# LongmaoTeamTf/deep_recommenders

Hardware: AMD Instinct MI355X
Metric: examples/sec/node DeepFM (26 sparse feats, 10M vocab, dim 64) (higher is better)
Workload: dtype f32; 1 GPU; DeepFM Criteo-shape synthetic training step (BASELINE.json configs[2]): 26 sparse + 13 dense, 10000000 vocab/field hashed on device, dim 64, DNN [256, 32]+[1] relu, sigmoid-CE, fused SGD; batch 65536 per GPU, ids uniform; tables on one GPU (66.6 GB); gemm_split=f16x2, global_batch=65536, parallelism=single, per_kernel_events=False

## Files before the change

deep_recommenders_amd/csrc/bf3_planes.hip:

```cpp
#include "bf3_rs_core.h"

namespace {

using namespace drrs;

constexpr int NWAVES = 8;
constexpr int NTHREADS = 64 * NWAVES;

struct NtArgs {
    const __bf16* A; int64_t a_ps, a_ld;
    const __bf16* B; int64_t b_ps, b_ld;
    int64_t M; int32_t N; int32_t K;
    float* C; int64_t ldc;
    const float* bias; int32_t act;
    const float* mask; int64_t ld_mask;
};


template <int NW, int DBG = 0>
__global__ __launch_bounds__(64 * NW, NW / 4) void bf3_gemm_nt_pipe_kernel(NtArgs g) {
    constexpr int BM = 128, BN = 128, NS = 3;
    constexpr int WN = 4, WM = NW / WN, TM = BM / (32 * WM);
    constexpr int A_PLANE = BM * 64, B_PLANE = BN * 64;
    constexpr int STAGE = 3 * (A_PLANE + B_PLANE);
    constexpr int KB_A = 3 * A_PLANE / 1024, PW = STAGE / 1024 / NW;
    constexpr int P1 = (PW + 1) / 2, P0 = PW - P1;
    static_assert((NW == 8 || NW == 16) && PW * NW * 1024 == STAGE, "wave layout");
    __shared__ __attribute__((aligned(1024))) unsigned char smem[NS * STAGE];

    const int tid = threadIdx.x, lane = tid & 63;
    const int wave = __builtin_amdgcn_readfirstlane(tid >> 6);
    const int wm = wave / WN, wn = wave % WN;
    const int l31 = lane & 31, hi = lane >> 5;

    const int tiles_n = (g.N + BN - 1) / BN;
    const int tiles_m = (int)((g.M + BM - 1) / BM);
    const int ntiles = tiles_m * tiles_n;
    const int nk = g.K / BK;
    if ((int)blockIdx.x >= ntiles) return;
    const int my_tiles = (ntiles - (int)blockIdx.x + (int)gridDim.x - 1) / (int)gridDim.x;
    const int total = my_tiles * nk;

    const unsigned lds0 = (unsigned)(uintptr_t)(lds_ptr_t)smem;
    const int sw = (l31 >> 2) & 3;
    unsigned a_addr[2], b_addr[2];
#pragma unroll
    for (int ks = 0; ks < 2; ++ks) {
        a_addr[ks] = lds0 + (wm * 32 * TM + l31) * 64 + (((2 * ks + hi) ^ sw) << 4);
        b_addr[ks] = lds0 + 3 * A_PLANE + (wn * 32 + l31) * 64 + (((2 * ks + hi) ^ sw) << 4);
    }

    const __bf16* src[PW];
    int p_tile = blockIdx.x, p_kt = 0, p_stage = 0;
    auto setup_src = [&](int tile) {
        const int lid = xcd_remap(tile, ntiles);
        const int64_t m0 = (int64_t)(lid / tiles_n) * BM;
        const int n0 = (lid % tiles_n) * BN;
#pragma unroll
        for (int i = 0; i < PW; ++i) {
            const int j = wave + NW * i;
            const bool is_a = j < KB_A;
            const int jj = is_a ? j : j - KB_A;
            const int plane = jj >> 3, rb = jj & 7;
            const int row = rb * 16 + (lane >> 2);
            const int c = (lane & 3) ^ ((row >> 2) & 3);
            int64_t grow = (is_a ? m0 : (int64_t)n0) + row;
            const int64_t lim = is_a ? g.M : (int64_t)g.N;
            grow = grow < lim ? grow : lim - 1;
            src[i] = is_a ? g.A + plane * g.a_ps + grow * g.a_ld + c * 8 : g.B + plane * g.b_ps + grow * g.b_ld + c * 8;
        }
    };
    auto issue_piece = [&](int i) {
        lds_dma16(src[i], smem + p_stage * STAGE + (wave + NW * i) * 1024);
        if constexpr (!(DBG & 4)) src[i] += BK;
    };
    auto advance = [&]() {
        p_stage = p_stage == NS - 1 ? 0 : p_stage + 1;
        if (++p_kt == nk) {
            p_kt = 0;
            p_tile += gridDim.x;
            if (p_tile < ntiles) setup_src(p_tile);
        }
    };
// ... 391 lines not shown
        const float4* s4 = reinterpret_cast<const float4*>(src);
        const int64_t stride = (int64_t)gridDim.x * blockDim.x;
        int64_t i = (int64_t)blockIdx.x * blockDim.x + threadIdx.x;
        for (; i + 3 * stride < nv; i += 4 * stride) {
            const float4 v0 = s4[i], v1 = s4[i + stride], v2 = s4[i + 2 * stride], v3 = s4[i + 3 * stride];
            take4(v0); take4(v1); take4(v2); take4(v3);
        }
        for (; i < nv; i += stride) take4(s4[i]);
        for (int64_t j = (nv << 2) + (int64_t)blockIdx.x * blockDim.x + threadIdx.x; j < n; j += stride) m = max(m, __float_as_uint(fabsf(src[j])));
    } else {
        const bool vec = al16 && (ld & 3) == 0;
        const int cv = vec ? (C >> 2) : 0;
        for (int64_t r = blockIdx.x; r < R; r += gridDim.x) {
            const float* row = src + r * ld;
            for (int c = threadIdx.x; c < cv; c += blockDim.x) take4(reinterpret_cast<const float4*>(row)[c]);
            for (int c = (cv << 2) + threadIdx.x; c < C; c += blockDim.x) m = max(m, __float_as_uint(fabsf(row[c])));
        }
    }
#pragma unroll
    for (int o = 32; o > 0; o >>= 1) m = max(m, (uint32_t)__shfl_xor((int)m, o, 64));
    __shared__ uint32_t wm[4];
    if ((threadIdx.x & 63) == 0) wm[threadIdx.x >> 6] = m;
    __syncthreads();
    if (threadIdx.x == 0) {
        m = max(max(wm[0], wm[1]), max(wm[2], wm[3]));
        if (m > __hip_atomic_load(amax, __ATOMIC_RELAXED, __HIP_MEMORY_SCOPE_AGENT)) atomicMax(amax, m);
    }
}

__global__ __launch_bounds__(256) void h2_split_kernel(const float* __restrict__ src, int64_t ld_src, int64_t R, int32_t C,
                                                       _Float16* __restrict__ planes, int64_t ps, int64_t ldp, int64_t r0,
                                                       int64_t c0, int32_t transpose, const uint32_t* __restrict__ amax) {
    float sc, inv;
    h2_scale_of(amax[0], sc, inv);
    h2_mode_on();
    const int64_t total = R * C, stride = (int64_t)gridDim.x * blockDim.x;
    if (!transpose && (C & 3) == 0 && (ldp & 3) == 0 && (c0 & 3) == 0 && (ld_src & 3) == 0 && (reinterpret_cast<uintptr_t>(src) & 15) == 0 &&
        (reinterpret_cast<uintptr_t>(planes) & 7) == 0 && (ps & 3) == 0 && total < (int64_t)0x7fffffff) {
        typedef _Float16 f16x4 __attribute__((ext_vector_type(4)));
        typedef float f32x4 __attribute__((ext_vector_type(4)));
        const unsigned cq = (unsigned)C >> 2, tq = (unsigned)(total >> 2);
        for (unsigned i = blockIdx.x * blockDim.x + threadIdx.x; i < tq; i += (unsigned)stride) {
            const unsigned r = i / cq, c = (i - r * cq) << 2;
            const f32x4 v = *reinterpret_cast<const f32x4*>(src + (int64_t)r * ld_src + c) * sc;
            const f16x4 h = __builtin_convertvector(v, f16x4);
            const f16x4 l = __builtin_convertvector(v - __builtin_convertvector(h, f32x4), f16x4);
            const int64_t off = (r0 + r) * ldp + c0 + c;
            *reinterpret_cast<f16x4*>(planes + off) = h;
            *reinterpret_cast<f16x4*>(planes + ps + off) = l;
        }
        return;
    }
    for (int64_t i = (int64_t)blockIdx.x * blockDim.x + threadIdx.x; i < total; i += stride) {
        int64_t r, c, off;
        if (!transpose) { r = i / C; c = i - r * C; off = (r0 + r) * ldp + c0 + c; }
        else { c = i / R; r = i - c * R; off = (r0 + c) * ldp + c0 + r; }
        const float v = src[r * ld_src + c] * sc;
        const _Float16 h = (_Float16)v;
        planes[off] = h;
        planes[ps + off] = (_Float16)(v - (float)h);
    }
}

constexpr int H2_REFRESH_PARTS = 256;
__global__ __launch_bounds__(256) void h2_amax_parts_kernel(const float* __restrict__ src, int64_t ld, int64_t R, int32_t C,
                                                            uint32_t* __restrict__ parts) {
    uint32_t m = 0u;
    const int64_t total = R * (int64_t)C, stride = (int64_t)gridDim.x * blockDim.x;
    for (int64_t i = (int64_t)blockIdx.x * blockDim.x + threadIdx.x; i < total; i += stride) {
        const int64_t r = i / C;
        m = max(m, __float_as_uint(fabsf(src[r * ld + (i - r * C)])));
    }
#pragma unroll
    for (int o = 32; o > 0; o >>= 1) m = max(m, (uint32_t)__shfl_xor((int)m, o, 64));
    __shared__ uint32_t wm[4];
    if ((threadIdx.x & 63) == 0) wm[threadIdx.x >> 6] = m;
    __syncthreads();
    if (threadIdx.x == 0) parts[blockIdx.x] = max(max(wm[0], wm[1]), max(wm[2], wm[3]));
}
__global__ __launch_bounds__(256) void h2_split_both_kernel(const float* __restrict__ src, int64_t ld, int64_t R, int32_t C,
                                                            _Float16* __restrict__ w, int64_t w_ps, int64_t w_ld,
                                                            _Float16* __restrict__ wt, int64_t wt_ps, int64_t wt_ld,
                                                            const uint32_t* __restrict__ parts, int32_t nparts, uint32_t* __restrict__ amax) {
    uint32_t m = (int)threadIdx.x < nparts ? parts[threadIdx.x] : 0u;
#pragma unroll
    for (int o = 32; o > 0; o >>= 1) m = max(m, (uint32_t)__shfl_xor((int)m, o, 64));
    __shared__ uint32_t wm[4];
    if ((threadIdx.x & 63) == 0) wm[threadIdx.x >> 6] = m;
    __syncthreads();
    m = max(max(wm[0], wm[1]), max(wm[2], wm[3]));
    if (blockIdx.x == 0 && threadIdx.x == 0) amax[0] = m;
    float sc, inv;
    h2_scale_of(m, sc, inv);
    h2_mode_on();
    const int64_t total = R * (int64_t)C, stride = (int64_t)gridDim.x * blockDim.x;
    for (int64_t i = (int64_t)blockIdx.x * blockDim.x + threadIdx.x; i < 2 * total; i += stride) {
        int64_t r, c, off;
        _Float16* dst;
        int64_t ps;
        if (i < total) { r = i / C; c = i - r * C; off = r * w_ld + c; dst = w; ps = w_ps; }
        else { const int64_t j = i - total; c = j / R; r = j - c * R; off = c * wt_ld + r; dst = wt; ps = wt_ps; }
        const float v = src[r * ld + c] * sc;
        const _Float16 h = (_Float16)v;
        dst[off] = h;
        dst[ps + off] = (_Float16)(v - (float)h);
    }
}

__global__ __launch_bounds__(256) void bf3_join_kernel(const __bf16* __restrict__ planes, int64_t ps, int64_t ldp, int64_t R,
                                                       int32_t C, float* __restrict__ dst, int64_t ld_dst) {
    const int64_t total = R * C, stride = (int64_t)gridDim.x * blockDim.x;
    for (int64_t i = (int64_t)blockIdx.x * blockDim.x + threadIdx.x; i < total; i += stride) {
        const int64_t r = i / C;
        const int c = (int)(i - r * C);
        const int64_t off = r * ldp + c;
        dst[r * ld_dst + c] = bf3::join(planes[off], planes[ps + off], planes[2 * ps + off]);
    }
}

}

extern "C" int dr_bf3_split(const float* src, int64_t ld_src, int64_t R, int32_t C, void* planes, int64_t plane_stride,
                            int64_t ld_planes, int64_t row_offset, int64_t col_offset, int32_t transpose,
                            dr_stream_t stream) {
    if (R < 0 || C < 0 || ld_src < C || row_offset < 0 || col_offset < 0 || ld_planes <= 0 || plane_stride <= 0) return DR_EINVAL;
    if (R == 0 || C == 0) return DR_OK;
    if (!src || !planes) return DR_EINVAL;
    if (!transpose && col_offset + C > ld_planes) return DR_EINVAL;
    if (transpose && col_offset + R > ld_planes) return DR_EINVAL;
    hipLaunchKernelGGL(bf3_split_kernel, dim3(dr_grid_for(R * ((C + 3) / 4), 256)), dim3(256), 0, dr_s(stream), src, ld_src, R, C,
                       static_cast<__bf16*>(planes), plane_stride, ld_planes, row_offset, col_offset, transpose);
    DR_CHECK_LAUNCH();
    return DR_OK;
}

extern "C" int dr_bf3_join(const void* planes, int64_t plane_stride, int64_t ld_planes, int64_t R, int32_t C, float* dst,
                           int64_t ld_dst, dr_stream_t stream) {
    if (R < 0 || C < 0 || ld_planes < C || ld_dst < C || plane_stride <= 0) return DR_EINVAL;
    if (R == 0 || C == 0) return DR_OK;
    if (!planes || !dst) return DR_EINVAL;
    hipLaunchKernelGGL(bf3_join_kernel, dim3(dr_grid_for(R * C, 256)), dim3(256), 0, dr_s(stream),
                       static_cast<const __bf16*>(planes), plane_stride, ld_planes, R, C, dst, ld_dst);
    DR_CHECK_LAUNCH();
    return DR_OK;
}

extern "C" int dr_bf3_gemm_nt(const void* a_planes, int64_t a_plane_stride, int64_t a_ld, const void* b_planes,
                              int64_t b_plane_stride, int64_t b_ld, int64_t M, int32_t N, int32_t K, const float* bias,
                              int32_t act, const float* mask, int64_t ld_mask, float* C, int64_t ldc, dr_stream_t stream) {
    if (M < 0 || N <= 0 || K <= 0 || (K % BK) != 0 || act < 0 || act > 1) return DR_EINVAL;
    if (M == 0) return DR_OK;
    if (!planes_ok(a_planes, a_plane_stride, a_ld) || !planes_ok(b_planes, b_plane_stride, b_ld) || !C) return DR_EINVAL;
    if (a_ld < K || b_ld < K || ldc < N || (mask != nullptr && ld_mask < N)) return DR_EINVAL;
    NtArgs g{static_cast<const __bf16*>(a_planes), a_plane_stride, a_ld, static_cast<const __bf16*>(b_planes), b_plane_stride, b_ld,
             M, N, K, C, ldc, bias, act, mask, ld_mask};
    const int64_t tiles = ((M + 127) / 128) * ((N + 127) / 128);
    if (tiles > 0x7fffffff) return DR_EINVAL;
    const int grid = (int)(tiles < 256 ? tiles : 256);
    hipLaunchKernelGGL((bf3_gemm_nt_pipe_kernel<16>), dim3(grid), dim3(1024), 0, dr_s(stream), g);
    DR_CHECK_LAUNCH();
    return DR_OK;
}

extern "C" int64_t dr_bf3_gemm_tn_workspace_bytes(int64_t R, int32_t F, int32_t N) {
    if (R <= 0 || F <= 0 || N <= 0) return 0;
    return (int64_t)tn_split_for(R, F, N, 128, 256) * F * N * (int64_t)sizeof(float);
}

extern "C" int dr_bf3_gemm_tn(const void* x_planes, int64_t x_plane_stride, int64_t x_ld, const void* y_planes,
                              int64_t y_plane_stride, int64_t y_ld, int64_t R, int32_t F, int32_t N, float scale, float* dst,
                              int64_t ld_dst, const float* y_colsum, float* dstb, void* workspace, int64_t workspace_bytes,
                              dr_stream_t stream) {
    if (R <= 0 || F <= 0 || N <= 0) return DR_EINVAL;
    if (!planes_ok(x_planes, x_plane_stride, x_ld) || !planes_ok(y_planes, y_plane_stride, y_ld) || !dst || !workspace) return DR_EINVAL;
    if (x_ld < F || y_ld < N || ld_dst < N) return DR_EINVAL;
    if (workspace_bytes < dr_bf3_gemm_tn_workspace_bytes(R, F, N)) return DR_EINVAL;
    TnArgs g{static_cast<const __bf16*>(x_planes), x_plane_stride, x_ld, static_cast<const __bf16*>(y_planes), y_plane_stride, y_ld,
             R, F, N, 0, 0, static_cast<float*>(workspace)};
    int split = tn_split_for(R, F, N, 128, 256);
    const int64_t rpad = (R + BK - 1) / BK * BK;
    g.per = ((rpad + split - 1) / split + BK - 1) / BK * BK;
    g.split = (int32_t)((rpad + g.per - 1) / g.per);
    const int64_t tiles = (int64_t)((F + 127) / 128) * ((N + 255) / 256) * g.split;
    const int grid = (int)(tiles < 256 ? tiles : 256);
    hipLaunchKernelGGL((bf3_gemm_tn_kernel<2, 4>), dim3(grid), dim3(NTHREADS), 0, dr_s(stream), g);
    hipLaunchKernelGGL(bf3_splitk_reduce_kernel, dim3(dr_grid_for((int64_t)F * N, 256)), dim3(256), 0, dr_s(stream), g.partial,
                       g.split, (int64_t)F, N, scale, dst, ld_dst, y_colsum, dstb);
    DR_CHECK_LAUNCH();
    return DR_OK;
// ... 40 lines not shown
```

deep_recommenders_amd/csrc/emb_plan.hip:

```cpp
#include "dr_common.h"
#include "hash_i64.h"
#include <atomic>

namespace {

constexpr int CH = 32;
constexpr uint32_t EMPTY = 0xFFFFFFFFu;
constexpr uint32_t DUPBIT = 0x80000000u;
constexpr int SMALL_CAP = 16384;
constexpr int RADIX_BITS = 8, RADIX = 1 << RADIX_BITS;
constexpr int NBK = RADIX, CAPB = 128;
constexpr int LDS_TAB_MAX_LOG = 15;
constexpr int RADIX_CHUNK = 1664, RADIX_MAX_BLOCKS = 1024;
constexpr int MARK_BLOCKS = 512, MARK_MAX_CHUNK = 8192;
static_assert(NBK * CAPB >= SMALL_CAP, "buckets must hold the largest SMALL list");

std::atomic<int> g_small_limit{SMALL_CAP};

struct Ctrl {
    int32_t large;
    int32_t pad[3];
    int32_t bcnt[NBK];
};

// ... 467 lines not shown
    __syncthreads();
    const uint32_t base_row = rmin;
    int passes = 0;
    if (cnt > 1 && rmax > rmin) passes = (int)((bits_for_dev(rmax - rmin) + RADIX_BITS - 1) / RADIX_BITS);
    if (passes & 1) {
        for (int32_t i = t; i < cnt; i += LG_T) dst[i] = src[i];
        uint64_t* x = src; src = dst; dst = x;
        __syncthreads();
    }
    for (int p = 0; p < passes; ++p) {
        const uint32_t shift = (uint32_t)(p * RADIX_BITS);
        if (t < RADIX) running[t] = 0;
        __syncthreads();
        for (int32_t i = t; i < cnt; i += LG_T)
            atomicAdd(&running[(((uint32_t)(src[i] >> 24) - base_row) >> shift) & (RADIX - 1)], 1u);
        __syncthreads();
        {
            const uint32_t mine = t < RADIX ? running[t] : 0u;
            for (int o = 1; o < RADIX; o <<= 1) {
                const uint32_t x = (t < RADIX && t >= o) ? running[t - o] : 0u;
                __syncthreads();
                if (t < RADIX) running[t] += x;
                __syncthreads();
            }
            if (t < RADIX) running[t] -= mine;
        }
        __syncthreads();
        for (int32_t base = 0; base < cnt; base += LG_T) {
            const int32_t i = base + t;
            const bool live = i < cnt;
            const uint64_t k = live ? src[i] : 0ull;
            scatter_step_1024(live, k, (((uint32_t)(k >> 24) - base_row) >> shift) & (RADIX - 1), running, wcnt, dst);
        }
        uint64_t* x = src; src = dst; dst = x;
    }
    for (int32_t base = 0; base < cnt; base += LG_T) {
        const int32_t i = base + t;
        const bool in = i < cnt;
        const uint64_t ck = in ? src[i] : ~0ull;
        const uint64_t k = ck >> 24;
        const int32_t gi = (int32_t)beg + i;
        const bool valid = in && k < num_rows;
        const bool seg_start = in && (i == 0 || (src[i - 1] >> 24) != k);
        const bool has_next = in && (i + 1 < cnt) && (src[i + 1] >> 24) == k;
        if (in) {
            const int32_t slot = (int32_t)(ck & 0xFFFFFFu);
            rows[gi] = k;
            slots[gi] = slot;
            flags[slot] = (valid && seg_start && !has_next) ? 1 : 0;
        }
        const bool head = valid && ((seg_start && has_next) || (!seg_start && (gi % CH) == 0 && i >= CH && (src[i - CH] >> 24) == k));
        if (t == 0) nh = 0;
        __syncthreads();
        const uint64_t bal = __ballot(head);
        int wbase = 0;
        const int leader = bal != 0 ? __ffsll((unsigned long long)bal) - 1 : 0;
        if (bal != 0 && lane == leader) wbase = atomicAdd(&nh, __popcll(bal));
        __syncthreads();
        if (t == 0) gbase = nh > 0 ? atomicAdd(dup_count, nh) : 0;
        __syncthreads();
        if (bal != 0) {
            wbase = __shfl(wbase, leader, 64);
            if (head) dup_heads[gbase + wbase + __popcll(bal & ((1ull << lane) - 1ull))] = gi;
        }
    }
}

}

extern "C" int32_t dr_emb_plan_set_small_limit(int32_t limit) {
    if (limit < 0) limit = 0;
    if (limit > SMALL_CAP) limit = SMALL_CAP;
    return g_small_limit.exchange(limit);
}

extern "C" int64_t dr_emb_sort_workspace_bytes(int64_t n) {
    if (n <= 0) return 256;
    return (int64_t)layout_for(n).total;
}

namespace {
int plan_small_front(const int64_t* raw, const uint64_t* col_buckets, int64_t* ids_out, int32_t* ids_t, const int64_t* ids, int64_t B,
                     int32_t F, const int64_t* row_base, int64_t num_rows, uint64_t* rows_y, uint64_t* keys_x, uint32_t* ghist,
                     uint32_t* tot, Ctrl* ctrl, int32_t* dup_count, hipStream_t s) {
    const int64_t n64 = B * F;
    const int32_t n = (int32_t)n64;
    const uint32_t mul = (uint32_t)((((uint64_t)RADIX) << 32) / (uint64_t)num_rows);
    int64_t sub = 64;
    while ((B + sub - 1) / sub > RADIX_MAX_BLOCKS) sub += 64;
    const int nbf = (int)((B + sub - 1) / sub);
    const int nbs = (nbf + FRONT_GROUP - 1) / FRONT_GROUP;
    const int64_t chunk = sub * FRONT_GROUP * F;
    if (chunk > 0x7fffffff) return DR_EINVAL;
    const bool trans = ids_t != nullptr;
    const size_t lds = (size_t)8 * (raw ? 3 : 1) * F + (trans ? (size_t)4 * 64 * (F + 1) : 0);
    if (raw) {
        if (trans)
            hipLaunchKernelGGL((plan_front_kernel<true, true>), dim3(nbf), dim3(256), lds, s, raw, B, F, col_buckets, ids_out, ids_t, row_base,
                               (uint64_t)num_rows, mul, (int32_t)sub, rows_y, ghist);
        else
            hipLaunchKernelGGL((plan_front_kernel<true, false>), dim3(nbf), dim3(256), lds, s, raw, B, F, col_buckets, ids_out, ids_t,
                               row_base, (uint64_t)num_rows, mul, (int32_t)sub, rows_y, ghist);
    } else {
        hipLaunchKernelGGL((plan_front_kernel<false, false>), dim3(nbf), dim3(256), lds, s, ids, B, F, col_buckets, ids_out, ids_t, row_base,
                           (uint64_t)num_rows, mul, (int32_t)sub, rows_y, ghist);
    }
    hipLaunchKernelGGL((radix_scan_kernel<true>), dim3(RADIX), dim3(256), 0, s, ghist, (int32_t)nbf, tot, ctrl, dup_count);
    hipLaunchKernelGGL(plan_scatter_kernel, dim3(nbs), dim3(LG_T), 0, s, rows_y, keys_x, n, mul, (int32_t)chunk, ghist, (int32_t)nbf, tot);
    return DR_OK;
}

int sort_slots_impl(const int64_t* raw, const uint64_t* col_buckets, int32_t* ids_t, const int64_t* ids, int64_t B, int32_t F,
                    const int64_t* row_base, int64_t num_rows, int64_t* sorted_rows, int32_t* sorted_slots, uint8_t* unique_flags,
                    int32_t* dup_heads, int32_t* dup_count, void* workspace, int64_t workspace_bytes, dr_stream_t stream) {
    if (B < 0 || F <= 0 || num_rows <= 0) return DR_EINVAL;
    const int64_t n64 = B * F;
    if (n64 == 0) return DR_OK;
    if (n64 > 0x7fffff00) return DR_EINVAL;
    if (!ids || !row_base || !sorted_rows || !sorted_slots || !unique_flags || !dup_heads || !dup_count || !workspace)
        return DR_EINVAL;
    if (workspace_bytes < dr_emb_sort_workspace_bytes(n64)) return DR_EINVAL;
    const int32_t n = (int32_t)n64;
    const Layout L = layout_for(n64);
    char* w = static_cast<char*>(workspace);
    uint64_t* keys_x = reinterpret_cast<uint64_t*>(w + L.keys_x);
    uint32_t* vals_x = reinterpret_cast<uint32_t*>(w + L.vals_x);
    uint64_t* blist = reinterpret_cast<uint64_t*>(w + L.blist);
    uint32_t* ghist = reinterpret_cast<uint32_t*>(w + L.ghist);
    uint32_t* tot = reinterpret_cast<uint32_t*>(w + L.tot);
    Ctrl* ctrl = reinterpret_cast<Ctrl*>(w + L.ctrl);
    uint64_t* rows_y = reinterpret_cast<uint64_t*>(sorted_rows);
    uint32_t* slots_y = reinterpret_cast<uint32_t*>(sorted_slots);
    hipStream_t s = dr_s(stream);
    const int grid = dr_grid_for(n, 256);
    const int nb = radix_blocks(n);

    const bool claimable = n64 <= (1 << 24) && num_rows < 0x7fffffffLL;
    const bool fused_front = raw != nullptr && claimable && F <= 64;
    if (raw && !fused_front) {
        int rc = dr_hash_bucket_i64(raw, B, F, col_buckets, const_cast<int64_t*>(ids), stream);
        if (rc == DR_OK && ids_t) rc = dr_ids_transpose_i32(ids, B, F, ids_t, stream);
        if (rc != DR_OK) return rc;
    }
    if (claimable) {
        int rc = plan_small_front(fused_front ? raw : nullptr, col_buckets, const_cast<int64_t*>(ids), fused_front ? ids_t : nullptr, ids, B,
                                  F, row_base, num_rows, rows_y, keys_x, ghist, tot, ctrl, dup_count, s);
        if (rc != DR_OK) return rc;
        static const hipError_t lds_optin = hipFuncSetAttribute(reinterpret_cast<const void*>(plan_lds_claim_kernel),
                                                                hipFuncAttributeMaxDynamicSharedMemorySize, 4 << LDS_TAB_MAX_LOG);
        if (lds_optin != hipSuccess) return DR_ELAUNCH;
        int log_tab = 12;
        while (log_tab < LDS_TAB_MAX_LOG && (1 << log_tab) < 2 * ((n + NBK - 1) / NBK)) ++log_tab;
        hipLaunchKernelGGL(plan_lds_claim_kernel, dim3(NBK), dim3(CLAIM_T), (size_t)4 << log_tab, s, keys_x, tot, (uint64_t)num_rows,
                           (int32_t)log_tab, unique_flags, blist, ctrl);
        hipLaunchKernelGGL(plan_bucket_sort_kernel, dim3(NBK), dim3(256), 0, s, blist, ctrl, (int32_t)g_small_limit.load(), rows_y,
                           sorted_slots, dup_heads, dup_count);
        hipLaunchKernelGGL(plan_large_kernel, dim3(NBK), dim3(LG_T), 0, s, keys_x, tot, (uint64_t)num_rows, n, rows_y, sorted_slots,
                           unique_flags, dup_heads, dup_count, ctrl);
        DR_CHECK_LAUNCH();
        return DR_OK;
    }
    if (hipMemsetAsync(dup_count, 0, 2 * sizeof(int32_t), s) != hipSuccess) return DR_ELAUNCH;
    const unsigned bits = bits_for((uint64_t)num_rows);
    const int passes = (int)((bits + RADIX_BITS - 1) / RADIX_BITS);
    uint64_t* kbuf[2] = {keys_x, rows_y};
    uint32_t* vbuf[2] = {vals_x, slots_y};
    int cur = (passes & 1) ? 0 : 1;
    hipLaunchKernelGGL(radix_make_keys_kernel, dim3(grid), dim3(256), 0, s, ids, n, F, row_base, (uint64_t)num_rows, kbuf[cur], vbuf[cur]);
    for (int p = 0; p < passes; ++p) {
        const uint32_t shift = (uint32_t)(p * RADIX_BITS);
        hipLaunchKernelGGL(radix_hist_kernel, dim3(nb), dim3(256), 0, s, kbuf[cur], n, shift, ghist);
        hipLaunchKernelGGL((radix_scan_kernel<false>), dim3(RADIX), dim3(256), 0, s, ghist, (int32_t)nb, tot, ctrl, dup_count);
        hipLaunchKernelGGL(radix_scatter_kernel, dim3(nb), dim3(256), 0, s, kbuf[cur], vbuf[cur], kbuf[cur ^ 1], vbuf[cur ^ 1], n, shift, ghist,
                           tot);
        cur ^= 1;
    }
    int mark_blocks = MARK_BLOCKS;
    while ((n + mark_blocks - 1) / mark_blocks > MARK_MAX_CHUNK) mark_blocks *= 2;
    hipLaunchKernelGGL(radix_mark_kernel, dim3(mark_blocks), dim3(256), 0, s, rows_y, sorted_slots, n, (uint64_t)num_rows, unique_flags, dup_heads,
                       dup_count);
    DR_CHECK_LAUNCH();
    return DR_OK;
}
}

extern "C" int dr_emb_sort_slots(const int64_t* ids, int64_t B, int32_t F, const int64_t* row_base, int64_t num_rows,
                                 int64_t* sorted_rows, int32_t* sorted_slots, uint8_t* unique_flags, int32_t* dup_heads,
                                 int32_t* dup_count, void* workspace, int64_t workspace_bytes, dr_stream_t stream) {
    return sort_slots_impl(nullptr, nullptr, nullptr, ids, B, F, row_base, num_rows, sorted_rows, sorted_slots, unique_flags, dup_heads,
                           dup_count, workspace, workspace_bytes, stream);
}

extern "C" int dr_hash_sort_slots(const int64_t* keys, int64_t B, int32_t F, const uint64_t* col_buckets, int64_t* ids_out,
                                  int32_t* ids_t_out, const int64_t* row_base, int64_t num_rows, int64_t* sorted_rows,
                                  int32_t* sorted_slots, uint8_t* unique_flags, int32_t* dup_heads, int32_t* dup_count, void* workspace,
                                  int64_t workspace_bytes, dr_stream_t stream) {
    if (!keys || !col_buckets || !ids_out) return DR_EINVAL;
    return sort_slots_impl(keys, col_buckets, ids_t_out, ids_out, B, F, row_base, num_rows, sorted_rows, sorted_slots, unique_flags,
                           dup_heads, dup_count, workspace, workspace_bytes, stream);
}
```

deep_recommenders_amd/csrc/emb_sorted.hip:

```cpp
#include <cstdlib>
#include "dr_common.h"
#include "tn_rs_reduce.h"
#include <hip/amd_detail/amd_hip_unsafe_atomics.h>
#include <cstring>

namespace {

constexpr int CH = 32;

#ifndef DR_K4_NT
#define DR_K4_NT 1
#endif
typedef float dr_f4v __attribute__((ext_vector_type(4)));
__device__ __forceinline__ float4 ld4_stream(const float* p) {
#if DR_K4_NT
    const dr_f4v v = __builtin_nontemporal_load(reinterpret_cast<const dr_f4v*>(p));
    return make_float4(v.x, v.y, v.z, v.w);
#else
    return *reinterpret_cast<const float4*>(p);
#endif
}
__device__ __forceinline__ void st4_stream(float* p, const float4 v) {
#if DR_K4_NT
    const dr_f4v w = {v.x, v.y, v.z, v.w};
// ... 242 lines not shown
        const bool exclusive = seg_start && (j >= n || rows[j < n ? j : n - 1] != k);
        float* dst = table + k * (uint64_t)D + sub * 4;
        if (ADAM) {
            if (live && seg_start) {
                if (dvalid) {
                    float4 t = *reinterpret_cast<const float4*>(dst);
                    float4 mt = *reinterpret_cast<const float4*>(ad.m + k * (uint64_t)D + sub * 4);
                    float4 vt = *reinterpret_cast<const float4*>(ad.v + k * (uint64_t)D + sub * 4);
                    t.x += adam_elem(g.x, mt.x, vt.x, ad); t.y += adam_elem(g.y, mt.y, vt.y, ad);
                    t.z += adam_elem(g.z, mt.z, vt.z, ad); t.w += adam_elem(g.w, mt.w, vt.w, ad);
                    wmax = amax4(wmax, t);
                    *reinterpret_cast<float4*>(dst) = t;
                    *reinterpret_cast<float4*>(ad.m + k * (uint64_t)D + sub * 4) = mt;
                    *reinterpret_cast<float4*>(ad.v + k * (uint64_t)D + sub * 4) = vt;
                }
                if (lin_w != nullptr && any_lin && sub == 0) {
                    float ml = ad.m_lin != nullptr ? ad.m_lin[k * ad.lin_stride] : 0.f, vl = ad.v_lin != nullptr ? ad.v_lin[k * ad.lin_stride] : 0.f;
                    lin_w[k] += adam_elem(dls, ml, vl, ad);
                    if (ad.m_lin != nullptr) { ad.m_lin[k * ad.lin_stride] = ml; ad.v_lin[k * ad.lin_stride] = vl; }
                }
            }
        } else if (live) {
            if (exclusive) {
                if (dvalid) {
                    float4 t = *reinterpret_cast<const float4*>(dst);
                    t.x = fmaf(scale, g.x, t.x); t.y = fmaf(scale, g.y, t.y);
                    t.z = fmaf(scale, g.z, t.z); t.w = fmaf(scale, g.w, t.w);
                    wmax = amax4(wmax, t);
                    *reinterpret_cast<float4*>(dst) = t;
                }
                if (lin_w != nullptr && any_lin && sub == 0) lin_w[k] = fmaf(scale, dls, lin_w[k]);
            } else if (det) {
                if (dvalid) *reinterpret_cast<float4*>(x_sorted + i * (int64_t)D + sub * 4) = g;
                if (any_lin && sub == 0 && j - i >= 2) x_sorted[(i + 1) * (int64_t)D] = dls;
            } else {
                if (dvalid && amax != nullptr) {
                    float4 o;
                    o.x = unsafeAtomicAdd(dst + 0, scale * g.x) + scale * g.x; o.y = unsafeAtomicAdd(dst + 1, scale * g.y) + scale * g.y;
                    o.z = unsafeAtomicAdd(dst + 2, scale * g.z) + scale * g.z; o.w = unsafeAtomicAdd(dst + 3, scale * g.w) + scale * g.w;
                    wmax = amax4(wmax, o);
                } else if (dvalid) {
                    unsafeAtomicAdd(dst + 0, scale * g.x); unsafeAtomicAdd(dst + 1, scale * g.y);
                    unsafeAtomicAdd(dst + 2, scale * g.z); unsafeAtomicAdd(dst + 3, scale * g.w);
                }
                if (lin_w != nullptr && any_lin && sub == 0) unsafeAtomicAdd(lin_w + k, scale * dls);
            }
        }
    }
    if (amax != nullptr) amax_commit(amax, wmax);
}

struct BwdSortedArgs {
    const int64_t* ids; const uint8_t* flags; int64_t B; int32_t F; const int64_t* row_base; int32_t D;
    const float* grad; int64_t ld; const float* concat; int64_t ldc; const float* sum_x; const float* d_fm_logit;
    const float* slot_lin; float scale; float* table; float* lin_w; float* lin_bias;
    const uint64_t* rows; const int32_t* slots; int64_t n; const int32_t* dup_heads; const int32_t* dup_count; uint64_t num_rows;
    float* x_sorted;
    int det;
    int skip_unique_lin;
    const float* lin_old_t;
    uint32_t* amax;
    int dups_only;
};
#ifndef DR_K4_MINWAVES
#define DR_K4_LB __launch_bounds__(256)
#else
#define DR_K4_LB __launch_bounds__(256, DR_K4_MINWAVES)
#endif
template <int LPR, int U, bool ADAM>
__global__ DR_K4_LB void emb_bwd_sorted_kernel(BwdSortedArgs a, AdamArgs ad, int grid_d) {
    if ((int)blockIdx.x < grid_d)
        emb_bwd_dups_body<LPR, ADAM>(blockIdx.x, grid_d, a.rows, a.slots, a.n, a.dup_heads, a.dup_count, a.F, a.D, a.num_rows, a.grad,
                                     a.ld, a.concat, a.ldc, a.sum_x, a.d_fm_logit, a.slot_lin, a.scale, a.table, a.lin_w, ad, a.x_sorted,
                                     a.det != 0, a.amax);
    else if (a.dups_only) {
        if (!ADAM && a.lin_bias != nullptr && a.d_fm_logit != nullptr) dr_block_sum_axpy(a.d_fm_logit, a.B, a.scale, a.lin_bias);
    } else
        emb_bwd_unique_body<LPR, U, ADAM>(blockIdx.x - grid_d, gridDim.x - grid_d, a.ids, a.flags, a.B, a.F, a.row_base, a.D, a.grad,
                                          a.ld, a.concat, a.ldc, a.sum_x, a.d_fm_logit, a.slot_lin, a.scale, a.table,
                                          a.skip_unique_lin ? nullptr : a.lin_w, a.lin_bias, ad, a.lin_old_t, a.amax);
}

template <int LPR>
__global__ __launch_bounds__(256) void emb_bwd_dups_apply_kernel(BwdSortedArgs a, drrs::TnRsApply ap, int grid_d) {
    const int bid = blockIdx.x;
    if (bid < grid_d)
        emb_bwd_dups_body<LPR, false>(bid, grid_d, a.rows, a.slots, a.n, a.dup_heads, a.dup_count, a.F, a.D, a.num_rows, a.grad, a.ld,
                                      a.concat, a.ldc, a.sum_x, a.d_fm_logit, a.slot_lin, a.scale, a.table, a.lin_w, AdamArgs{}, a.x_sorted,
                                      a.det != 0, a.amax);
    else if (bid == grid_d) {
        if (a.lin_bias != nullptr && a.d_fm_logit != nullptr) dr_block_sum_axpy(a.d_fm_logit, a.B, a.scale, a.lin_bias);
    } else
        drrs::tn_rs_reduce_ride(ap, bid - grid_d - 1, (int)gridDim.x - grid_d - 1, threadIdx.x);
}

template <int LPR>
__global__ __launch_bounds__(256) void emb_bwd_hot_apply_kernel(BwdSortedArgs a) {
    constexpr int NS = DR_WAVE / LPR;
    const int lane = threadIdx.x & 63, grp = lane / LPR, sub = lane % LPR;
    const int D = a.D, F = a.F;
    const bool dvalid = sub < (D >> 2);
    const int subc = dvalid ? sub : (D >> 2) - 1;
    const bool any_lin = a.lin_w != nullptr && (a.d_fm_logit != nullptr || a.slot_lin != nullptr);
    const int64_t nwaves = (int64_t)gridDim.x * (blockDim.x >> 6);
    const int64_t wave0 = (int64_t)blockIdx.x * (blockDim.x >> 6) + (threadIdx.x >> 6);
    const int64_t nheads = a.dup_count[0], n = a.dup_count[1];
    float wmax = 0.f;
    constexpr int SCREEN = 16;
    for (int64_t h0 = wave0 * SCREEN; h0 < nheads; h0 += nwaves * SCREEN) {
        const int64_t h = h0 + lane;
        int64_t my_i = 0, my_stop = 0;
        bool hot = false;
        if (lane < SCREEN && h < nheads) {
            my_i = a.dup_heads[h];
            const uint64_t k = a.rows[my_i];
            const bool seg_start = (my_i == 0) || (a.rows[my_i - 1] != k);
            my_stop = ((my_i % CH) == 0) ? my_i + CH : ((my_i + CH - 1) / CH + 1) * CH;
            hot = seg_start && my_stop < n && a.rows[my_stop] == k;
        }
        uint64_t todo = __ballot(hot);
        while (todo != 0ull) {
            const int src = __ffsll((unsigned long long)todo) - 1;
            todo &= todo - 1ull;
            const int64_t i = __shfl(my_i, src, 64), stop = __shfl(my_stop, src, 64);
            const uint64_t k = a.rows[i];
            int64_t np = 0;
            for (;;) {
                const int64_t pos = stop + (np + lane) * CH;
                const bool ok = pos < n && a.rows[pos < n ? pos : n - 1] == k;
                const uint64_t m = __ballot(ok);
                const int c = m == ~0ull ? 64 : (__ffsll((unsigned long long)~m) - 1);
                np += c;
                if (c < 64) break;
            }
            const int64_t lp = stop + (np - 1) * CH;
            int64_t e;
            {
                const int64_t pos = lp + lane;
                const bool ok = lane < CH && pos < n && a.rows[pos < n ? pos : n - 1] == k;
                const uint64_t m = __ballot(ok);
                e = lp + (__ffsll((unsigned long long)~m) - 1);
            }
            const int64_t P = np + 1, per = (P + NS - 1) / NS;
            const int64_t q0 = grp * per, q1 = (q0 + per < P) ? q0 + per : P;
            float4 g = make_float4(0.f, 0.f, 0.f, 0.f);
            for (int64_t q = q0; q < q1; q += 4) {
                float4 v[4];
#pragma unroll
                for (int u = 0; u < 4; ++u) {
                    const int64_t qq = (q + u < q1) ? q + u : q1 - 1;
                    const int64_t pos = qq == 0 ? i : stop + (qq - 1) * CH;
                    v[u] = *reinterpret_cast<const float4*>(a.x_sorted + pos * (int64_t)D + subc * 4);
                }
#pragma unroll
                for (int u = 0; u < 4; ++u)
                    if (q + u < q1) { g.x += v[u].x; g.y += v[u].y; g.z += v[u].z; g.w += v[u].w; }
            }
#pragma unroll
            for (int o = 1; o < NS; ++o) {
                const float ox = __shfl(g.x, sub + o * LPR, 64), oy = __shfl(g.y, sub + o * LPR, 64);
                const float oz = __shfl(g.z, sub + o * LPR, 64), ow = __shfl(g.w, sub + o * LPR, 64);
                if (grp == 0) { g.x += ox; g.y += oy; g.z += oz; g.w += ow; }
            }
            if (grp == 0 && dvalid) {
                float* dst = a.table + k * (uint64_t)D + sub * 4;
                float4 t = *reinterpret_cast<const float4*>(dst);
                t.x = fmaf(a.scale, g.x, t.x); t.y = fmaf(a.scale, g.y, t.y);
                t.z = fmaf(a.scale, g.z, t.z); t.w = fmaf(a.scale, g.w, t.w);
                wmax = amax4(wmax, t);
                *reinterpret_cast<float4*>(dst) = t;
            }
            if (any_lin) {
                float dls = 0.f;
                for (int64_t q = lane; q < P; q += 64) {
                    const int64_t pos = q == 0 ? i : stop + (q - 1) * CH;
                    const bool single = q == P - 1 && e - pos < 2;
                    float v = a.x_sorted[(single ? pos : pos + 1) * (int64_t)D];
                    if (single) {
                        const int32_t sp = a.slots[pos];
                        v = a.slot_lin != nullptr ? a.slot_lin[sp] : a.d_fm_logit[sp / F];
                    }
                    dls += v;
                }
#pragma unroll
                for (int off = 32; off > 0; off >>= 1) dls += __shfl_xor(dls, off, 64);
                if (lane == 0) a.lin_w[k] = fmaf(a.scale, dls, a.lin_w[k]);
            }
        }
    }
    if (a.amax != nullptr) amax_commit(a.amax, wmax);
}

}

static int bwd_sorted_impl(const int64_t* ids, const int64_t* row_base, const int64_t* sorted_rows,
                           const int32_t* sorted_slots, const uint8_t* unique_flags, const int32_t* dup_heads,
                           const int32_t* dup_count, int64_t B, int32_t F, int32_t D, int64_t num_rows, const float* grad,
                           int64_t ld_grad, const float* concat, int64_t ld_concat, const float* sum_x,
                           const float* d_fm_logit, const float* slot_lin_grad, float scale, float* dst_table,
                           float* dst_lin, float* dst_bias, const AdamArgs* adam, float* x_sorted, dr_stream_t stream,
                           int parts, const float* lin_old_t, uint32_t* table_amax, const drrs::TnRsApply* apply = nullptr) {
    if (B < 0 || F <= 0 || F > 64 || D < 4 || D > 256 || (D & 3) || num_rows <= 0) return DR_EINVAL;
    const int64_t n = B * F;
    if (n == 0) return DR_OK;
    if (!ids || !row_base || !sorted_rows || !sorted_slots || !unique_flags || !dup_heads || !dup_count || !grad ||
        !dst_table ||
        ld_grad < (int64_t)F * D || (ld_grad & 3))
        return DR_EINVAL;
    if (concat != nullptr && (ld_concat < (int64_t)F * D || (ld_concat & 3) || sum_x == nullptr)) return DR_EINVAL;
    if (sum_x != nullptr && d_fm_logit == nullptr) return DR_EINVAL;
    if (sum_x != nullptr && concat == nullptr && x_sorted == nullptr) return DR_EINVAL;
    int lpr = 1;
    while (lpr * 4 < D) lpr <<= 1;
    const uint64_t* rows = reinterpret_cast<const uint64_t*>(sorted_rows);
    const int grid_u = dr_grid_for(B, 4, 8192);
    const int grid_d = 2048;
    AdamArgs ad{};
    if (adam != nullptr) ad = *adam;
    static const bool det_on = [] { const char* e = getenv("DR_K4_DETERMINISTIC"); return !(e != nullptr && e[0] == '0'); }();
    const int det = (adam == nullptr && x_sorted != nullptr && det_on) ? 1 : 0;
    const BwdSortedArgs ba{ids, unique_flags, B, F, row_base, D, grad, ld_grad, concat, ld_concat, sum_x, d_fm_logit, slot_lin_grad,
                           scale, dst_table, dst_lin, dst_bias, rows, sorted_slots, n, dup_heads, dup_count, (uint64_t)num_rows,
                           x_sorted, det, (adam == nullptr && (parts & 4)) ? 1 : 0,
                           slot_lin_grad == nullptr ? lin_old_t : nullptr, table_amax, (parts & 8) ? 1 : 0};
#ifdef DR_K4_U
    constexpr int K4_U_OVERRIDE = DR_K4_U;
#else
    constexpr int K4_U_OVERRIDE = 0;
#endif
    const int nlb = apply != nullptr ? drrs::tn_rs_reduce_blocks(apply->F, apply->N, apply->vec) : 0;
    const int riders = nlb < 1024 ? nlb : 1024;
#define LAUNCH(L, ADAM_)                                                                                              \
    { if (apply != nullptr) {                                                                                         \
        hipLaunchKernelGGL((emb_bwd_dups_apply_kernel<L>), dim3(grid_d + 1 + riders), dim3(256), 0, dr_s(stream), ba, *apply, grid_d);     \
    } else {                                                                                                          \
        constexpr int NS_ = 64 / L;                                                                                   \
        constexpr int U_ = K4_U_OVERRIDE > 0 ? K4_U_OVERRIDE : (NS_ >= 16 ? 2 : 4);                                   \
        hipLaunchKernelGGL((emb_bwd_sorted_kernel<L, U_, ADAM_>), dim3(grid_d + ((parts & 8) ? 1 : grid_u)), dim3(256), 0, dr_s(stream), ba, ad,    \
                           grid_d);                                                                                   \
    } }
#define CALL(L)                                                                                                       \
    if (adam != nullptr) LAUNCH(L, true) else LAUNCH(L, false)
    if (parts & 1)
    switch (lpr) {
        case 1: CALL(1); break;
        case 2: CALL(2); break;
        case 4: CALL(4); break;
        case 8: CALL(8); break;
        case 16: CALL(16); break;
        case 32: CALL(32); break;
        case 64: CALL(64); break;
        default: return DR_EINVAL;
    }
#undef CALL
#undef LAUNCH
    DR_CHECK_LAUNCH();
    if (det && (parts & 2)) {
#define HOT(L) hipLaunchKernelGGL((emb_bwd_hot_apply_kernel<L>), dim3(1024), dim3(256), 0, dr_s(stream), ba)
        switch (lpr) {
            case 1: HOT(1); break;
            case 2: HOT(2); break;
            case 4: HOT(4); break;
            case 8: HOT(8); break;
            case 16: HOT(16); break;
            case 32: HOT(32); break;
            default: HOT(64); break;
        }
#undef HOT
        DR_CHECK_LAUNCH();
    }
    return DR_OK;
}

extern "C" int dr_emb_pool_bwd_sorted(const int64_t* ids, const int64_t* row_base, const int64_t* sorted_rows,
                                      const int32_t* sorted_slots, const uint8_t* unique_flags,
                                      const int32_t* dup_heads, const int32_t* dup_count, int64_t B, int32_t F,
                                      int32_t D, int64_t num_rows, const float* grad, int64_t ld_grad,
                                      const float* concat, int64_t ld_concat, const float* sum_x,
                                      const float* d_fm_logit, const float* slot_lin_grad, float scale,
                                      float* dst_table, float* dst_lin, float* dst_bias, float* x_sorted,
                                      const float* lin_old_t, int32_t parts, uint32_t* table_amax, dr_stream_t stream) {
    if (parts < 1 || parts > 15 || (parts & 3) == 0) return DR_EINVAL;
    return bwd_sorted_impl(ids, row_base, sorted_rows, sorted_slots, unique_flags, dup_heads, dup_count, B, F, D, num_rows,
                           grad, ld_grad, concat, ld_concat, sum_x, d_fm_logit, slot_lin_grad, scale, dst_table, dst_lin,
                           dst_bias, nullptr, x_sorted, stream, parts, lin_old_t, table_amax);
}

extern "C" int dr_emb_pool_bwd_dups_apply(const int64_t* ids, const int64_t* row_base, const int64_t* sorted_rows,
                                          const int32_t* sorted_slots, const uint8_t* unique_flags, const int32_t* dup_heads,
                                          const int32_t* dup_count, int64_t B, int32_t F, int32_t D, int64_t num_rows, const float* grad,
                                          int64_t ld_grad, const float* sum_x, const float* d_fm_logit, float scale, float* dst_table,
                                          float* dst_lin, float* dst_bias, float* x_sorted, const float* lin_old_t, int32_t parts,
                                          uint32_t* table_amax, void* wg_workspace, int64_t wg_workspace_bytes, int64_t wg_R, int32_t wg_F,
                                          int32_t wg_N, int32_t wg_h2, float wg_scale, float* dstW, int64_t ld_w, float* dstb,
                                          dr_stream_t stream) {
    if (parts != 9 && parts != 11) return DR_EINVAL;
    if (wg_R <= 0 || wg_F <= 0 || wg_N <= 0 || !wg_workspace || !dstW || ld_w < wg_N) return DR_EINVAL;
    if (wg_workspace_bytes < dr_bf3_wgrad_workspace_bytes(wg_R, wg_F, wg_N)) return DR_EINVAL;
    if (B <= 0) return DR_EINVAL;
    int split, Fp, Np;
    int64_t per;
    drrs::tn_rs_plan(wg_R, wg_F, wg_N, split, per, Fp, Np);
    const drrs::TnRsApply ap = drrs::tn_rs_apply_of(wg_workspace, split, wg_F, wg_N, Fp, Np, wg_h2 != 0, wg_scale, dstW, ld_w, dstb);
    return bwd_sorted_impl(ids, row_base, sorted_rows, sorted_slots, unique_flags, dup_heads, dup_count, B, F, D, num_rows, grad, ld_grad,
                           nullptr, 0, sum_x, d_fm_logit, nullptr, scale, dst_table, dst_lin, dst_bias, nullptr, x_sorted, stream, parts,
                           lin_old_t, table_amax, &ap);
}

namespace {
__global__ __launch_bounds__(256) void lin_update_unique_kernel(const int64_t* __restrict__ ids, const uint8_t* __restrict__ flags,
                                                                int64_t n, int32_t F, const int64_t* __restrict__ row_base,
                                                                const float* __restrict__ d_fm_logit,
                                                                const float* __restrict__ slot_lin, float scale,
                                                                float* __restrict__ lin_w) {
    const int64_t stride = (int64_t)gridDim.x * blockDim.x;
    for (int64_t s = (int64_t)blockIdx.x * blockDim.x + threadIdx.x; s < n; s += stride) {
        const int64_t id = ids[s];
        if (id < 0 || !flags[s]) continue;
        const int64_t b = s / F;
        const int f = (int)(s - b * F);
        const int64_t row = row_base[f] + id;
        const float g = slot_lin != nullptr ? slot_lin[s] : d_fm_logit[b];
        lin_w[row] = fmaf(scale, g, lin_w[row]);
    }
}
}

extern "C" int dr_emb_lin_update_unique(const int64_t* ids, const uint8_t* unique_flags, int64_t B, int32_t F,
                                        const int64_t* row_base, const float* d_fm_logit, const float* slot_lin_grad, float scale,
                                        float* dst_lin, dr_stream_t stream) {
    if (B < 0 || F <= 0 || F > 64) return DR_EINVAL;
    if (B == 0) return DR_OK;
    if (!ids || !unique_flags || !row_base || !dst_lin || (!d_fm_logit && !slot_lin_grad)) return DR_EINVAL;
    const int64_t n = B * F;
    hipLaunchKernelGGL(lin_update_unique_kernel, dim3(dr_grid_for(n, 256, 4096)), dim3(256), 0, dr_s(stream), ids, unique_flags, n, F,
                       row_base, d_fm_logit, slot_lin_grad, scale, dst_lin);
    DR_CHECK_LAUNCH();
    return DR_OK;
}

namespace {
__global__ __launch_bounds__(256) void snapshot_sorted_rows_kernel(const uint64_t* __restrict__ rows, const int32_t* __restrict__ dup_heads,
                                                                   const int32_t* __restrict__ dup_count, const float* __restrict__ table,
                                                                   int32_t D, uint64_t num_rows, float* __restrict__ x_sorted) {
    const int64_t nh = dup_count[0];
    const int q = D >> 2;
    const int64_t total = nh * q, stride = (int64_t)gridDim.x * blockDim.x;
    for (int64_t t = (int64_t)blockIdx.x * blockDim.x + threadIdx.x; t < total; t += stride) {
        const int64_t h = t / q;
        const int c = (int)(t - h * q);
        const int64_t i = dup_heads[h];
        const uint64_t k = rows[i];
        float4 v = make_float4(0.f, 0.f, 0.f, 0.f);
        if (k < num_rows) v = *reinterpret_cast<const float4*>(table + k * (uint64_t)D + c * 4);
        *reinterpret_cast<float4*>(x_sorted + i * (int64_t)D + c * 4) = v;
    }
}
}

extern "C" int dr_emb_snapshot_sorted_rows(const int64_t* sorted_rows, const int32_t* dup_heads, const int32_t* dup_count,
                                           const float* table, int32_t D, int64_t num_rows, float* x_sorted, dr_stream_t stream) {
    if (D < 4 || (D & 3) || num_rows <= 0) return DR_EINVAL;
    if (!sorted_rows || !dup_heads || !dup_count || !table || !x_sorted) return DR_EINVAL;
    hipLaunchKernelGGL(snapshot_sorted_rows_kernel, dim3(1024), dim3(256), 0, dr_s(stream), reinterpret_cast<const uint64_t*>(sorted_rows),
                       dup_heads, dup_count, table, D, (uint64_t)num_rows, x_sorted);
    DR_CHECK_LAUNCH();
    return DR_OK;
}

extern "C" int dr_emb_pool_bwd_sorted_adam(const int64_t* ids, const int64_t* row_base, const int64_t* sorted_rows,
                                           const int32_t* sorted_slots, const uint8_t* unique_flags,
                                           const int32_t* dup_heads, const int32_t* dup_count, int64_t B, int32_t F,
                                           int32_t D, int64_t num_rows, const float* grad, int64_t ld_grad,
                                           const float* concat, int64_t ld_concat, const float* sum_x,
                                           const float* d_fm_logit, const float* slot_lin_grad, float lr_t, float beta1,
                                           float beta2, float eps, float* table, float* m_table, float* v_table,
                                           float* lin_w, float* m_lin, float* v_lin, float* x_sorted, const float* lin_old_t,
                                           uint32_t* table_amax, dr_stream_t stream) {
    if (!m_table || !v_table) return DR_EINVAL;
    if (lin_w != nullptr && (!m_lin || !v_lin)) return DR_EINVAL;
    AdamArgs ad{m_table, v_table, m_lin, v_lin, (m_lin != nullptr && v_lin == m_lin + 1) ? 2 : 1, lr_t, beta1, beta2, eps};
    return bwd_sorted_impl(ids, row_base, sorted_rows, sorted_slots, unique_flags, dup_heads, dup_count, B, F, D, num_rows,
                           grad, ld_grad, concat, ld_concat, sum_x, d_fm_logit, slot_lin_grad, 0.f, table, lin_w, nullptr,
                           &ad, x_sorted, stream, 3, lin_old_t, table_amax);
}

__global__ __launch_bounds__(256) void adam_catchup_rows_kernel(const int64_t* __restrict__ ids, int64_t n, int32_t F,
                                                                const int64_t* __restrict__ row_base, int32_t D,
                                                                float* __restrict__ table, float* __restrict__ m,
// ... 147 lines not shown
```

deep_recommenders_amd/csrc/tn_rs_reduce.h:

```cpp
#pragma once
#include "rs_args.h"

namespace drrs {

constexpr int TN_RS_HDR_WORDS = 4;
constexpr int TN_RS_RED_THREADS = 256;

struct TnRsApply {
    const float* partial; const float* colsum;
    const uint32_t* hdr;
    int32_t split, F, N, Fp, Np;
    float scale;
    float* dst; int64_t ld; float* dstb;
    int32_t vec;
};

__host__ __device__ inline int tn_rs_reduce_blocks(int F, int N, int vec) {
    const int w = vec ? (N + 3) / 4 : N;
    return (int)(((int64_t)F * w + TN_RS_RED_THREADS - 1) / TN_RS_RED_THREADS);
}

template <int V>
__device__ __forceinline__ void tn_rs_reduce_block(const TnRsApply& a, int lb, int tid) {
    typedef float vec_t __attribute__((ext_vector_type(V)));
    const int w = (a.N + V - 1) / V;
    const int64_t t = (int64_t)lb * TN_RS_RED_THREADS + tid;
    const int f = (int)(t / w);
    const int n = (int)(t - (int64_t)f * w) * V;
    if (f >= a.F) return;
    const int split = a.split, N = a.N, Np = a.Np;
    const int64_t ps = (int64_t)a.Fp * Np;
    float wscale = a.scale;
    if (a.hdr != nullptr) {
        float sx, ix, sy, iy;
        h2_scale_of(a.hdr[0], sx, ix);
        h2_scale_of(a.hdr[1], sy, iy);
        wscale = a.scale * (ix * iy);
    }
    auto sum_slices = [&](const float* p, int64_t stride) -> vec_t {
        vec_t acc = 0.f;
        int s = 0;
        for (; s + 8 <= split; s += 8) {
            vec_t v[8];
#pragma unroll
            for (int u = 0; u < 8; ++u) v[u] = *reinterpret_cast<const vec_t*>(p + (s + u) * stride);
#pragma unroll
            for (int u = 0; u < 8; ++u) acc += v[u];
        }
        for (; s < split; ++s) acc += *reinterpret_cast<const vec_t*>(p + s * stride);
        return acc;
    };
    const vec_t acc = sum_slices(a.partial + (int64_t)f * Np + n, ps);
    float* d = a.dst + (int64_t)f * a.ld + n;
    if (V == 1 || n + V <= N) {
        vec_t o = *reinterpret_cast<vec_t*>(d);
#pragma unroll
        for (int c = 0; c < V; ++c) o[c] = fmaf(wscale, acc[c], o[c]);
        *reinterpret_cast<vec_t*>(d) = o;
    } else {
#pragma unroll
        for (int c = 0; c < V; ++c)
            if (n + c < N) d[c] = fmaf(wscale, acc[c], d[c]);
    }
    if (f == 0 && a.colsum != nullptr && a.dstb != nullptr) {
        const vec_t cacc = sum_slices(a.colsum + n, Np);
#pragma unroll
        for (int c = 0; c < V; ++c)
            if (n + c < N) a.dstb[n + c] = fmaf(a.scale, cacc[c], a.dstb[n + c]);
    }
}

__device__ __forceinline__ void tn_rs_reduce_ride(const TnRsApply& a, int rider, int nriders, int tid) {
    const int nlb = tn_rs_reduce_blocks(a.F, a.N, a.vec);
    for (int lb = rider; lb < nlb; lb += nriders) {
        if (a.vec) tn_rs_reduce_block<4>(a, lb, tid);
        else tn_rs_reduce_block<1>(a, lb, tid);
    }
}

inline TnRsApply tn_rs_apply_of(void* workspace, int split, int32_t F, int32_t N, int Fp, int Np, bool h2, float scale, float* dst,
                                int64_t ld, float* dstb) {
    float* partial = static_cast<float*>(workspace);
    float* colsum = partial + (int64_t)split * Fp * Np;
    const uint32_t* hdr = reinterpret_cast<const uint32_t*>(colsum + (int64_t)split * Np);
    const bool vec = ((reinterpret_cast<uintptr_t>(partial) | reinterpret_cast<uintptr_t>(dst)) & 15) == 0 && (ld & 3) == 0;
    return TnRsApply{partial, dstb != nullptr ? colsum : nullptr, h2 ? hdr : nullptr, split, F, N, Fp, Np, scale, dst, ld, dstb, vec ? 1 : 0};
}

void tn_rs_plan(int64_t R, int32_t F, int32_t N, int& split, int64_t& per, int& Fp, int& Np);

}
```

deep_recommenders_amd/engine.py:

```python
import math
import os
from typing import List, Optional, Sequence

import torch

from . import ops
from .ops import _pad4


_SIDE_STREAMS = {}


def _side_streams(device):
    key = str(torch.device(device))
    if key not in _SIDE_STREAMS:
        _SIDE_STREAMS[key] = (torch.cuda.Stream(device=device), torch.cuda.Stream(device=device))
    return _SIDE_STREAMS[key]


class DeepFMEngine:
    def __init__(self, num_fields: int, vocab_per_field: int, dim: int, dnn_units: Sequence[int], batch: int,
                 num_dense: int = 0, lr: float = 0.01, device="cuda", seed: int = 42, hashed: bool = True,
                 table_init_std: Optional[float] = None, lin_init_std: float = 0.0, sorted_bwd: bool = True,
                 optimizer: str = "sgd", beta1: float = 0.9, beta2: float = 0.999, eps: float = 1e-8):
# ... 86 lines not shown
        self.concat = torch.zeros((B, self.ld), **f32)
        self.sum_x = torch.empty((B, D), **f32)
        self.fm_logit = torch.empty((B,), **f32)
        self.hs = [torch.empty((B, _pad4(u)), **f32)[:, :u] for u in units]
        self.dhs = [torch.empty((B, _pad4(u)), **f32)[:, :u] for u in units[:-1]]
        self.d_concat = torch.empty((B, self.ld), **f32)
        self.prob = torch.empty((B,), **f32)
        self.d_logit = torch.empty((B,), **f32)
        self.loss = torch.zeros(1, **f32)
        self.ws = torch.empty(1024, **f32)
        self._events = None
        self._ev_every, self._ev_step, self._ev_live = 1, 0, False
        self._ev_pool = []
        self._ev_only = None
        self.sorted_bwd = sorted_bwd
        self.fuse_k3 = os.environ.get("DR_FUSE_K3", "1") == "1" and D == 64 and self.Nd <= 32 and V <= (1 << 24)
        self._dense_pads = ([torch.zeros((B, 32), dtype=torch.float32, device=device) for _ in range(2)]
                            if (self.fuse_k3 and self.Nd) else None)
        self._dense_amaxs = None
        self.no_concat = (os.environ.get("DR_NO_CONCAT", "1") == "1" and self.fuse_k3 and self.wplanes[0] is not None
                          and self.wg_ws[0] is not None and sorted_bwd and self.acts[0] in (0, 1) and len(dnn_units) >= 1
                          and not (self.fuse_head and len(self.Ws) == 2) and V < (1 << 24) - 1)
        if self.no_concat:
            self._ids_t = [torch.empty((F, B), dtype=torch.int32, device=device) for _ in range(2)]
            self.x_sorted = torch.empty((B * F, D), dtype=torch.float32, device=device)
        self.lin_old_t = (torch.empty((F, B), dtype=torch.float32, device=device)
                          if (self.fuse_k3 and sorted_bwd) else None)
        self._lin_old_valid = False
        self.h2 = (ops.get_gemm_split() == "f16x2" and self.no_concat and self.wplanes[0] is not None
                   and not self.adam_tf and os.environ.get("DR_OVERLAP_DW", "0") != "1")
        if self.h2:
            self.wplanes[0] = ops.H2WeightPlanes(self.Ws[0], double_buffer=True)
            self.tab_amax = ops.h2_amax(self.table)
            self._tab_ver = (self.table.data_ptr(), self.table._version)
            self._dense_amaxs = [ops.h2_record(device) for _ in range(2)] if self._dense_pads is not None else None
            self.dh0_amax = ops.h2_record(device)
            self._amax_scratch = ops.h2_record(device)
        self.tail_in_fwd = (os.environ.get("DR_TAIL_IN_FWD", "1") != "0" and self.h2 and self.fuse_k3 and self.fuse_tail and nl == 3
                            and optimizer == "sgd"
                            and ops.h2_emb_linear_tail_supported(B, self.Ws[0].shape[1], self.Ws[1].shape[1]))
        self.fwd_tail_ws = ops.h2_emb_linear_tail_workspace(B, device) if self.tail_in_fwd else None
        self._tail_in_fwd_ran = False
        self._tighten_every = int(os.environ.get("DR_AMAX_TIGHTEN_STEPS", "2048"))
        self._steps_since_tighten = 0
        _pe = os.environ.get("DR_PREFETCH_EARLY", "2")
        self.prefetch_early = _pe in ("1", "2")
        self.prefetch_after_fwd = _pe == "2" and self.fuse_k3
        self._plan_prefetched = False
        if sorted_bwd:
            self._plans = [ops.SortPlan(B * F, device) for _ in range(2)]
            self.side, self.side_r = _side_streams(device)
            self._refresh_stream = self.side
            self.ev_ids = torch.cuda.Event()
            self._ev_sorted = [torch.cuda.Event(), torch.cuda.Event()]
            self._ev_hashed = [torch.cuda.Event(), torch.cuda.Event()]
            self.ev_k4 = torch.cuda.Event()
            self.ev_dw_done = torch.cuda.Event()
            self.ev_planes = torch.cuda.Event()
            self.ev_dlogit = torch.cuda.Event()
            self.ev_lin = torch.cuda.Event()
            self.ev_fwd0 = torch.cuda.Event()
            self.ev_part1 = torch.cuda.Event()
            self.ev_small = torch.cuda.Event()
            self._ev_dense = [torch.cuda.Event(), torch.cuda.Event()]
            self._dense_by_event = False
        self.lin_side = (sorted_bwd and optimizer == "sgd" and os.environ.get("DR_LIN_SIDE", "0") == "1")
        self._k4_det = not os.environ.get("DR_K4_DETERMINISTIC", "1").startswith("0")
        self.fuse_k4 = (os.environ.get("DR_FUSE_K4", "1") != "0" and self.h2 and optimizer == "sgd" and sorted_bwd and self.no_concat
                        and D == 64 and not self.lin_side and self.lin_old_t is not None
                        and self.Ws[0].shape[0] >= F * D)
        _rs = os.environ.get("DR_REDUCE_SIDE", "0")
        self.reduce_side = sorted_bwd and optimizer == "sgd" and _rs in ("1", "2")
        self.reduce_side_wgrad = self.reduce_side and _rs == "1" and not self.h2
        self._small_pending = False
        self._planes_pending = False
        self._planes_pending_l0 = False
        self._k4_fused_done = False
        self._in_train_step = False
        self._early_issued = False
        _ov = os.environ.get("DR_OVERLAP_DW", "0")
        self.overlap_dw = _ov == "1"
        if self.overlap_dw:
            self.no_concat = False
        self.fold_reduces = (os.environ.get("DR_FOLD_REDUCES", "1") != "0" and self.tail_in_fwd and self.fuse_k4 and self.h2
                             and optimizer == "sgd" and not self.overlap_dw and not self.reduce_side)
        self.concurrent = {}
        if self.overlap_dw:
            k4 = "emb_pool_bwd_adam" if optimizer == "adam" else "emb_pool_bwd"
            self.concurrent = {"linear_bwd_dw_L0": k4, k4: "linear_bwd_dw_L0"}
            self.side2 = torch.cuda.Stream(device=device)
            self.ev_dx = torch.cuda.Event()
            self.ev_dw = torch.cuda.Event()

    @property
    def dense_pad(self):
        return self._dense_pads[self.cur] if self._dense_pads is not None else None

    @property
    def dense_amax(self):
        return self._dense_amaxs[self.cur] if self._dense_amaxs is not None else None

    @property
    def ids(self):
        return self._ids[self.cur]

    @property
    def plan(self):
        return self._plans[self.cur]

    @property
    def ev_sorted(self):
        return self._ev_sorted[self.cur]

    @staticmethod
    def _token(keys):
        return (keys.data_ptr(), keys._version, tuple(keys.shape))

    def _prefetch_mark(self):
        nk = self._next_keys
        if nk is None or not self.sorted_bwd:
            return None
        ordered = self._planes_pending and self._planes_pending_l0
        if not ordered:
            self.ev_k4.record()
        return (ordered,)

    def _prefetch_issue(self, mark):
        if mark is None:
            return
        (ordered,) = mark
        nk = self._next_keys
        nxt = self.cur ^ 1
        early_done = self._early_issued
        self._early_issued = False
        st = self._refresh_stream if (early_done and ordered) else self.side
        nk.record_stream(st)
        with torch.cuda.stream(st):
            if not ordered:
                st.wait_event(self.ev_k4)
            if not early_done:
                self._k("next_batch: hash_bucket_i64(side stream, overlapped)", "overlap", self.B * self.F * 16,
                        lambda: ops.hash_bucket_i64(nk, self.col_buckets, out=self._ids[nxt]))
                if self.no_concat:
                    ops.ids_transpose_i32(self._ids[nxt], out=self._ids_t[nxt])
            nd = self._next_dense
            self._pref_dense = None
            if early_done and getattr(self, "_dense_early", False):
                self._pref_dense = self._token(nd)
            elif nd is not None and self.Nd and not self.overlap_dw:
                nd.record_stream(st)
                if not self.no_concat:
                    self.concat[:, self.F * self.D:self.F * self.D + self.Nd].copy_(nd)
                if self._dense_pads is not None:
                    self._dense_pads[nxt][:, :self.Nd].copy_(nd)
                    if self.h2:
                        ops.h2_amax(self._dense_pads[nxt], self._dense_amaxs[nxt])
                self._pref_dense = self._token(nd)
            if early_done and getattr(self, "_dense_early", False):
                self._dense_by_event = True
            elif early_done:
                self._ev_dense[nxt].record(st)
                self._dense_by_event = True
            else:
                self._dense_by_event = False
                self._ev_hashed[nxt].record(st)
                self._k("next_batch: emb_sort_slots(side stream, overlapped)", "overlap", self.B * self.F * 36,
                        lambda: ops.emb_sort_slots(self._ids[nxt], self.row_base, self.R, self._plans[nxt]))
                self._ev_sorted[nxt].record(st)
        self._pref = self._token(nk)

    def _prefetch_early(self):
        nk = self._next_keys
        self._early_issued = False
        if nk is None or not (self.prefetch_early and self.sorted_bwd):
            return
        nxt = self.cur ^ 1
        self.ev_fwd0.record()
        nk.record_stream(self.side)
        nd = self._next_dense
        self._dense_early = (nd is not None and self.Nd and self.no_concat and self._dense_pads is not None and not self.overlap_dw)
        if self._dense_early:
            nd.record_stream(self.side_r)
            with torch.cuda.stream(self.side_r):
                self.side_r.wait_event(self.ev_fwd0)
                self._dense_pads[nxt][:, :self.Nd].copy_(nd)
                if self.h2:
                    ops.h2_amax(self._dense_pads[nxt], self._dense_amaxs[nxt])
                self._ev_dense[nxt].record(self.side_r)
        with torch.cuda.stream(self.side):
            self.side.wait_event(self.ev_fwd0)
            self._k("next_batch: hash_sort_slots(side stream, overlapped)", "overlap", self.B * self.F * 52,
                    lambda: ops.hash_sort_slots(nk, self.col_buckets, self.row_base, self.R, self._ids[nxt],
                                                self._ids_t[nxt] if self.no_concat else None, self._plans[nxt]))
            self._ev_hashed[nxt].record(self.side)
            self._ev_sorted[nxt].record(self.side)
        self._early_issued = True

    def enable_kernel_events(self, on: bool, every: int = 1, only=None):
        self._ev_only = set(only) if only is not None else None
        for rec in (getattr(self, "_events", None) or {}).values():
            self._ev_pool.extend(rec[2])
        self._events = {} if on else None
        self._ev_every = max(1, int(every))
        self._ev_step = 0
        self._ev_live = bool(on)

    def reserve_kernel_events(self, n_pairs: int):
        while len(self._ev_pool) < n_pairs:
            self._ev_pool.append((torch.cuda.Event(enable_timing=True), torch.cuda.Event(enable_timing=True)))

    def _k(self, name, bound, work, fn):
        if self._events is None or not self._ev_live or (self._ev_only is not None and name not in self._ev_only):
            return fn()
        s, e = self._ev_pool.pop() if self._ev_pool else (torch.cuda.Event(enable_timing=True), torch.cuda.Event(enable_timing=True))
        s.record()
        r = fn()
        e.record()
        self._events.setdefault(name, [bound, work, []])[2].append((s, e))
        return r

    def kernel_event_summary(self):
        torch.cuda.synchronize()
        out = {}
        for name, (bound, work, evs) in (self._events or {}).items():
            ms = sum(s.elapsed_time(e) for s, e in evs) / len(evs)
            out[name] = {"bound": bound, "ms": ms, "n": len(evs),
                         "alg_bytes" if bound in ("hbm", "overlap") else "alg_flops": work}
            if name in getattr(self, "concurrent", {}):
                out[name]["concurrent_with"] = self.concurrent[name]
        return out

    def concurrent_pair_summary(self):
        torch.cuda.synchronize()
        done, out = set(), []
        for a, b in getattr(self, "concurrent", {}).items():
            if a in done or b in done or a not in (self._events or {}) or b not in (self._events or {}):
                continue
            done.update((a, b))
            ea, eb = self._events[a][2], self._events[b][2]
            n = min(len(ea), len(eb))
            tot = 0.0
            for (sa, fa), (sb, fb) in zip(ea[-n:], eb[-n:]):
                first = sa if sa.elapsed_time(sb) >= 0 else sb
                tot += max(first.elapsed_time(fa), first.elapsed_time(fb))
            out.append({"kernels": [a, b], "joint_us": tot / n * 1e3})
        return out

    def _wgrad_reduce_deferred(self, i):
        return self.reduce_side_wgrad and i == 0 and self.no_concat and self.wplanes[0] is not None and not self.overlap_dw

    def _side_part2(self, fn):
        self.ev_part1.record()
        with torch.cuda.stream(self.side):
            self.side.wait_event(self.ev_part1)
            fn()
            self.ev_small.record(self.side)
        self._small_pending = True

    def _wgrad(self, i, x, dy, sc, dstW, dstb, main_only=False):
        if i == 0 and self.h2:
            ops.h2_wgrad_emb(self._ids_t[self.cur], self.row_base, self.table, self.tab_amax, self.dense_pad, self.dense_amax, dy,
                             self.dh0_amax, sc, dstW, dstb, workspace=self.wg_ws[0],
                             parts=1 if (main_only or self._wgrad_reduce_deferred(i)) else 3)
        elif i == 0 and self.no_concat:
            ops.bf3_wgrad_emb(self._ids_t[self.cur], self.row_base, self.table, self.dense_pad, dy, sc, dstW, dstb,
                              workspace=self.wg_ws[0], parts=1 if self._wgrad_reduce_deferred(i) else 3)
        elif self.wg_ws[i] is not None:
            ops.bf3_wgrad(x, dy, sc, dstW, dstb, workspace=self.wg_ws[i])
        else:
            ops.linear_bwd_dw(x, dy, sc, dstW, dstb, workspace=self.dw_ws[i])

    def forward(self, keys: torch.Tensor, dense: Optional[torch.Tensor], labels: Optional[torch.Tensor],
                loss_mode: int = ops.LOSS_SIGMOID_CE):
        F, D = self.F, self.D
        B = self.B
        if self.optimizer == "adam":
            self.flat_grads.zero_()
# ... 190 lines not shown
                dy = None
                continue
            if i == 0 and self.h2:
                if not (n > 1 and self.narrow_ws[1] is not None):
                    ops.h2_amax(dy, self.dh0_amax)
                self._k("linear_bwd_dx_L%d" % i, "mfma", fl,
                        lambda dy=dy, rs=rs, dx=dx, i=i: ops.h2_linear_nt(dy, self.dh0_amax, self.wplanes[i].w, mask=rs, out=dx))
            elif self.wplanes[i] is not None:
                self._k("linear_bwd_dx_L%d" % i, "mfma", fl,
                        lambda dy=dy, rs=rs, dx=dx, i=i: ops.bf3_linear_nt(dy, self.wplanes[i].w, mask=rs, out=dx))
            else:
                self._k("linear_bwd_dx_L%d" % i, "mfma", fl,
                        lambda dy=dy, W=W, rs=rs, dx=dx: ops.linear_bwd_dx(dy, W, relu_src=rs, out=dx))
            if i == 0 and self.sorted_bwd and self._plan_prefetched:
                torch.cuda.current_stream().wait_event(self.ev_sorted)
            if i == 0 and self.overlap_dw:
                self.ev_dx.record()
                with torch.cuda.stream(self.side2):
                    self.side2.wait_event(self.ev_dx)
                    self._k("linear_bwd_dw_L%d" % i, "mfma", fl,
                            lambda x=x, dy=dy, i=i, dstW=dstW, dstb=dstb: self._wgrad(i, x, dy, sc, dstW, dstb))
                    if self.wplanes[i] is not None and not adam:
                        self.wplanes[i].refresh()
                    self.ev_dw.record(self.side2)
                dy = dx
                continue
            self._k("linear_bwd_dw_L%d" % i, "mfma", fl,
                    lambda x=x, dy=dy, i=i, dstW=dstW, dstb=dstb: self._wgrad(i, x, dy, sc, dstW, dstb))
            if self.wplanes[i] is not None and not adam:
                if self.sorted_bwd:
                    self.ev_dw_done.record()
                    self._refresh_stream = self.side
                    with torch.cuda.stream(self.side):
                        self.side.wait_event(self.ev_dw_done)
                        if self._wgrad_reduce_deferred(i) and self.h2:
                            ops.h2_wgrad_emb(self._ids_t[self.cur], self.row_base, self.table, self.tab_amax, self.dense_pad, self.dense_amax,
                                             dy, self.dh0_amax, sc, dstW, dstb, workspace=self.wg_ws[0], parts=2)
                        elif self._wgrad_reduce_deferred(i):
                            ops.bf3_wgrad_emb(self._ids_t[self.cur], self.row_base, self.table, self.dense_pad, dy, sc, dstW, dstb,
                                              workspace=self.wg_ws[0], parts=2)
                        self.wplanes[i].refresh()
                        self.ev_planes.record(self.side)
                    self._planes_pending = True
                    self._planes_pending_l0 = (i == 0)
                else:
                    self.wplanes[i].refresh()
            dy = dx
        if adam:
            self._adam_finish()
        elif self._k4_fused_done:
            self._k4_fused_done = False
        elif self.sorted_bwd:
            if not self._plan_prefetched:
                torch.cuda.current_stream().wait_event(self.ev_sorted)
            if self.no_concat and not self._k4_det:
                ops.emb_snapshot_sorted_rows(self.plan, self.table, self.R, self.x_sorted)
            mark = self._prefetch_mark()
            k4 = lambda parts: ops.emb_pool_bwd_sorted(self.ids, self.row_base, self.plan, D, self.R, self.d_concat, self.d_logit,
                                                       -lr, self.table, self.lin_w, self.lin_bias,
                                                       concat=None if self.no_concat else self.concat, sum_x=self.sum_x,
                                                       x_sorted=self.x_sorted if self.no_concat else None, parts=parts,
                                                       lin_old_t=self.lin_old_t if (self._lin_old_valid and not lin_side) else None,
                                                       table_amax=self.tab_amax if self.h2 else None)
            sk = 4 if lin_side else 0
            self._k("emb_pool_bwd", "hbm", self.alg_bytes_bwd() - (self.B * self.F * 8 if lin_side else 0),
                    lambda: k4(1 | sk))
            if self.no_concat:
                self._k("emb_hot_rows_apply", "hbm", 0, lambda: k4(2 | sk))
            if lin_side:
                torch.cuda.current_stream().wait_event(self.ev_lin)
            self._prefetch_issue(mark)
        else:
            self._k("emb_pool_bwd", "hbm", self.alg_bytes_bwd(),
                    lambda: ops.emb_pool_bwd(self.ids, F, self.col_start, self.row_base, D, self.d_concat, self.concat,
                                             self.sum_x, self.d_logit, -lr, self.table, self.lin_w, self.lin_bias))
        if self._small_pending:
            torch.cuda.current_stream().wait_event(self.ev_small)
            self._small_pending = False
        if self.overlap_dw and not adam:
            torch.cuda.current_stream().wait_event(self.ev_dw)

    def _backward_l0_fused_k4(self, x, dy, sc, dstW, dstb, fl):
        lr = self.lr
        torch.cuda.current_stream().wait_event(self.ev_sorted)
        fold = self.fold_reduces
        self._k("linear_bwd_dw_L0", "mfma", fl, lambda: self._wgrad(0, x, dy, sc, dstW, dstb, main_only=fold))
        w_old = self.wplanes[0].w
        early = self._early_issued
        rs = self.side_r if (early or fold) else self.side

        def refresh_planes_behind():
            self._refresh_stream = rs
            self.ev_dw_done.record()
            with torch.cuda.stream(rs):
                rs.wait_event(self.ev_dw_done)
                self.wplanes[0].refresh()
                self.ev_planes.record(rs)
            self._planes_pending = True
            self._planes_pending_l0 = True

        if not fold:
            refresh_planes_behind()
        mark = self._prefetch_mark()
        if early:
            self._prefetch_issue(mark)
        if not self._k4_det:
            ops.emb_snapshot_sorted_rows(self.plan, self.table, self.R, self.x_sorted)
        work = self.alg_bytes_bwd() - 4.0 * self.B * self.F * self.D + 4.0 * self.B * dy.shape[1]
        self._k("emb_pool_bwd_fused_dgrad_L0", "hbm", work,
                lambda: ops.h2_dgrad_emb_sgd(dy, self.dh0_amax, w_old, self._ids_t[self.cur], self.plan, self.row_base, self.table,
                                             self.lin_w, self.lin_old_t, self.sum_x, self.d_logit, -lr, self.d_concat, table_amax=self.tab_amax))
        k4 = lambda parts: ops.emb_pool_bwd_sorted(self.ids, self.row_base, self.plan, self.D, self.R, self.d_concat, self.d_logit, -lr,
                                                   self.table, self.lin_w, self.lin_bias, sum_x=self.sum_x, x_sorted=self.x_sorted,
                                                   parts=parts | 8, lin_old_t=self.lin_old_t, table_amax=self.tab_amax)
        if fold:
            self._k("emb_pool_bwd_dups", "hbm", 0,
                    lambda: ops.emb_pool_bwd_dups_apply(self.ids, self.row_base, self.plan, self.D, self.R, self.d_concat, self.d_logit, -lr,
                                                        self.table, self.lin_w, self.lin_bias, self.sum_x, self.x_sorted, self.lin_old_t,
                                                        self.tab_amax, self.wg_ws[0], self.B, sc, dstW, dstb, wg_h2=True, parts=1))
            refresh_planes_behind()
        else:
            self._k("emb_pool_bwd_dups", "hbm", 0, lambda: k4(1))
        self._k("emb_hot_rows_apply", "hbm", 0, lambda: k4(2))
        if not early:
            self._prefetch_issue(mark)
        self._k4_fused_done = True

    def _launch_sort(self):
        self.ev_ids.record()
        with torch.cuda.stream(self.side):
            self.side.wait_event(self.ev_ids)
            self._k("emb_sort_slots(side stream, overlapped)", "overlap", self.B * self.F * 36,
                    lambda: ops.emb_sort_slots(self.ids, self.row_base, self.R, self.plan))
            self.ev_sorted.record(self.side)

    def _adam_finish(self):
        self.t += 1
        lr_t = ops.adam_lr_t(self.lr, self.beta1, self.beta2, self.t)
        if not self._plan_prefetched:
            torch.cuda.current_stream().wait_event(self.ev_sorted)
        if self.no_concat:
            ops.emb_snapshot_sorted_rows(self.plan, self.table, self.R, self.x_sorted)
        mark = self._prefetch_mark()
        self._k("emb_pool_bwd_adam", "hbm", self.B * (28 * self.F * self.D + 40 * self.F),
                lambda: ops.emb_pool_bwd_sorted_adam(self.ids, self.row_base, self.plan, self.D, self.R, self.d_concat,
                                                     self.d_logit, lr_t, self.beta1, self.beta2, self.eps, self.table,
                                                     self.m_table, self.v_table, self.lin_w, self.m_lin, self.v_lin,
                                                     concat=None if self.no_concat else self.concat, sum_x=self.sum_x,
                                                     x_sorted=self.x_sorted if self.no_concat else None,
                                                     lin_old_t=self.lin_old_t if self._lin_old_valid else None,
                                                     table_amax=self.tab_amax if self.h2 else None))
        self._prefetch_issue(mark)
        ops.reduce_sum(self.d_logit, out=self.g_lin_bias)
        if self.overlap_dw:
            torch.cuda.current_stream().wait_event(self.ev_dw)
        self._k("adam_step_dense", "hbm", 28.0 * self.flat_params.numel(),
                lambda: ops.adam_step(self.flat_params, self.flat_grads, self.flat_m, self.flat_v, lr_t, self.beta1, self.beta2,
                                      self.eps))
        for wp in self.wplanes:
            if wp is not None:
                wp.refresh()

    def adam_flush(self):
        assert self.adam_tf
        V, F = self.V, self.F
        step = 1 << 20
        for v0 in range(0, V, step):
            v1 = min(V, v0 + step)
            ids = torch.arange(v0, v1, device=self.table.device, dtype=torch.int64)[:, None].expand(v1 - v0, F).contiguous()
            ops.adam_catchup_rows(ids, self.row_base, self.table, self.m_table, self.v_table, self.lin_w, self.m_lin, self.v_lin,
                                  self.row_step, self.t, self.t, self.lr, self.beta1, self.beta2, self.eps)

    def refresh_planes(self):
        for wp in self.wplanes:
            if wp is not None:
                wp.refresh()

    def train_step(self, keys, dense, labels, next_keys=None, next_dense=None):
        self._next_keys, self._next_dense = next_keys, next_dense
        if self._events is not None:
            self._ev_live = (self._ev_step % self._ev_every) == 0
            self._ev_step += 1
        self._in_train_step = True
        try:
            self.forward(keys, dense, labels)
            self.backward_and_update()
        finally:
            self._in_train_step = False
        self._next_keys = self._next_dense = None
        if self.h2 and self._tighten_every > 0:
            self._steps_since_tighten += 1
            if self._steps_since_tighten >= self._tighten_every:
                self.tighten_amax()
        return self.loss

    def tighten_amax(self):
        if not self.h2:
            return
        ops.h2_amax(self.table, self._amax_scratch)
        self.tab_amax.copy_(self._amax_scratch)
        self._steps_since_tighten = 0

    def alg_bytes_fwd(self):
        return self.B * (8 * self.F * self.D + 12 * self.F + 8)

    def alg_bytes_bwd(self):
# ... 9 lines not shown
```

deep_recommenders_amd/ops.py:

```python
from typing import Optional, Sequence

import torch

from . import _lib
from ._lib import check, lib, ptr, stream_ptr


def _c(t: torch.Tensor, dtype) -> torch.Tensor:
    if t.dtype != dtype:
        raise TypeError("expected %s, got %s" % (dtype, t.dtype))
    return t if t.is_contiguous() else t.contiguous()


def hash_bucket_i64(keys: torch.Tensor, col_buckets: torch.Tensor, out: Optional[torch.Tensor] = None):
    keys = _c(keys, torch.int64)
    B, C = keys.shape
    col_buckets = _c(col_buckets, torch.int64)
    assert col_buckets.numel() == C
    if out is None:
        out = torch.empty_like(keys)
    check(lib().dr_hash_bucket_i64(ptr(keys), B, C, ptr(col_buckets), ptr(out), stream_ptr()), "dr_hash_bucket_i64")
    return out


# ... 419 lines not shown
        counts = torch.empty(world, dtype=torch.int64, device=dev)
    if send_rows is None:
        send_rows = torch.empty(n, dtype=torch.int64, device=dev)
    if pos is None:
        pos = torch.empty((B, C), dtype=torch.int64, device=dev)
    if workspace is None:
        nbytes = lib().dr_shard_bucket_workspace_bytes(n, world)
        workspace = torch.empty(nbytes // 8, dtype=torch.int64, device=dev)
    check(lib().dr_shard_bucket_ids(ptr(ids), ptr(rep), n, C, int(rows_per_shard), int(world), ptr(counts), ptr(send_rows),
                                    ptr(pos), ptr(workspace), stream_ptr()), "dr_shard_bucket_ids")
    return counts, send_rows, pos


def rows_gather(rows, table, lin_w=None, out_rows=None, out_lin=None):
    rows = _c(rows, torch.int64)
    n = rows.numel()
    if table.dtype != torch.float32 or table.dim() != 2 or not table.is_contiguous():
        raise ValueError("rows_gather: table must be contiguous fp32 [R, D], got %s %s with strides %s"
                         % (table.dtype, tuple(table.shape), tuple(table.stride())))
    R, D = table.shape
    lin_w = _dense_arg(lin_w, "rows_gather: lin_w", numel=R, copy=False)
    if out_rows is None:
        out_rows = torch.empty((n, D), dtype=torch.float32, device=rows.device)
    elif out_rows.dtype != torch.float32 or not out_rows.is_contiguous() or out_rows.numel() < n * D:
        raise ValueError("rows_gather: out_rows must be contiguous fp32 with room for %s, got %s %s" % ((n, D), out_rows.dtype, tuple(out_rows.shape)))
    if out_lin is None and lin_w is not None:
        out_lin = torch.empty(n, dtype=torch.float32, device=rows.device)
    elif out_lin is not None and (out_lin.dtype != torch.float32 or not out_lin.is_contiguous() or out_lin.numel() < n):
        raise ValueError("rows_gather: out_lin must be contiguous fp32 with room for %d, got %s %s" % (n, out_lin.dtype, tuple(out_lin.shape)))
    check(lib().dr_rows_gather(ptr(rows), n, ptr(table), D, ptr(lin_w), ptr(out_rows), ptr(out_lin), stream_ptr()),
          "dr_rows_gather")
    return out_rows, out_lin


def rows_scatter_add(rows, grads, lin_grads, scale, table, lin_w):
    rows = _c(rows, torch.int64)
    n = rows.numel()
    if table.dtype != torch.float32 or table.dim() != 2 or not table.is_contiguous():
        raise ValueError("rows_scatter_add: table must be contiguous fp32 [R, D], got %s %s with strides %s"
                         % (table.dtype, tuple(table.shape), tuple(table.stride())))
    R, D = table.shape
    grads = _dense_arg(grads, "rows_scatter_add: grads", shape=(n, D))
    lin_grads = _dense_arg(lin_grads, "rows_scatter_add: lin_grads", numel=n)
    lin_w = _dense_arg(lin_w, "rows_scatter_add: lin_w", numel=R, copy=False)
    check(lib().dr_rows_scatter_add(ptr(rows), n, ptr(grads), D, ptr(lin_grads), float(scale), ptr(table), ptr(lin_w),
                                    stream_ptr()), "dr_rows_scatter_add")


def axpy(alpha, x, y):
    assert x.is_contiguous() and y.is_contiguous() and x.numel() == y.numel()
    check(lib().dr_axpy(x.numel(), float(alpha), ptr(x), ptr(y), stream_ptr()), "dr_axpy")


def emb_sort_workspace(n, device):
    return torch.empty(lib().dr_emb_sort_workspace_bytes(int(n)), dtype=torch.uint8, device=device)


class SortPlan:

    def __init__(self, n, device):
        self.n = int(n)
        self.rows = torch.empty(n, dtype=torch.int64, device=device)
        self.slots = torch.empty(n, dtype=torch.int32, device=device)
        self.flags = torch.empty(n, dtype=torch.uint8, device=device)
        self.dup_heads = torch.empty(n, dtype=torch.int32, device=device)
        self.dup_count = torch.zeros(4, dtype=torch.int32, device=device)
        self.workspace = emb_sort_workspace(n, device)

    def sorted_len(self):
        return int(self.dup_count[1].item())


def emb_sort_slots(ids, row_base, num_rows, plan=None):
    ids = _c(ids, torch.int64)
    B, F = ids.shape
    if plan is None or plan.n < B * F:
        plan = SortPlan(B * F, ids.device)
    check(lib().dr_emb_sort_slots(ptr(ids), B, F, ptr(row_base), int(num_rows), ptr(plan.rows), ptr(plan.slots),
                                  ptr(plan.flags), ptr(plan.dup_heads), ptr(plan.dup_count), ptr(plan.workspace),
                                  plan.workspace.numel(), stream_ptr()), "dr_emb_sort_slots")
    return plan


def hash_sort_slots(keys, col_buckets, row_base, num_rows, ids_out, ids_t_out=None, plan=None):
    keys = _c(keys, torch.int64)
    B, F = keys.shape
    assert ids_out.shape == (B, F) and ids_out.dtype == torch.int64 and ids_out.is_contiguous()
    if ids_t_out is not None:
        assert ids_t_out.shape == (F, B) and ids_t_out.dtype == torch.int32 and ids_t_out.is_contiguous()
    if plan is None or plan.n < B * F:
        plan = SortPlan(B * F, keys.device)
    check(lib().dr_hash_sort_slots(ptr(keys), B, F, ptr(col_buckets), ptr(ids_out), ptr(ids_t_out), ptr(row_base), int(num_rows),
                                   ptr(plan.rows), ptr(plan.slots), ptr(plan.flags), ptr(plan.dup_heads), ptr(plan.dup_count),
                                   ptr(plan.workspace), plan.workspace.numel(), stream_ptr()), "dr_hash_sort_slots")
    return plan


def emb_plan_set_small_limit(limit):
    return int(lib().dr_emb_plan_set_small_limit(int(limit)))


def emb_snapshot_sorted_rows(plan, table, num_rows, out):
    assert out.is_contiguous() and out.shape[0] >= plan.n and out.shape[1] == table.shape[1]
    check(lib().dr_emb_snapshot_sorted_rows(ptr(plan.rows), ptr(plan.dup_heads), ptr(plan.dup_count), ptr(table), table.shape[1],
                                            int(num_rows), ptr(out), stream_ptr()), "dr_emb_snapshot_sorted_rows")
    return out


def ids_transpose_i32(ids, out=None):
    ids = _c(ids, torch.int64)
    B, F = ids.shape
    if out is None:
        out = torch.empty((F, B), dtype=torch.int32, device=ids.device)
    check(lib().dr_ids_transpose_i32(ptr(ids), B, F, ptr(out), stream_ptr()), "dr_ids_transpose_i32")
    return out


def emb_pool_bwd_sorted(ids, row_base, plan, D, num_rows, grad, d_fm_logit, scale, dst_table, dst_lin=None, dst_bias=None,
                        concat=None, sum_x=None, slot_lin_grad=None, x_sorted=None, parts=3, lin_old_t=None, table_amax=None):
    ids = _c(ids, torch.int64)
    B, F = ids.shape
    assert grad.stride(1) == 1
    assert lin_old_t is None or (lin_old_t.shape == (F, B) and lin_old_t.is_contiguous() and lin_old_t.dtype == torch.float32)
    check(lib().dr_emb_pool_bwd_sorted(ptr(ids), ptr(row_base), ptr(plan.rows), ptr(plan.slots), ptr(plan.flags),
                                       ptr(plan.dup_heads), ptr(plan.dup_count), B, F, D, int(num_rows), ptr(grad),
                                       grad.stride(0), ptr(concat), concat.stride(0) if concat is not None else 0,
                                       ptr(sum_x), ptr(d_fm_logit), ptr(slot_lin_grad), float(scale), ptr(dst_table), ptr(dst_lin),
                                       ptr(dst_bias), ptr(x_sorted), ptr(lin_old_t), int(parts), ptr(table_amax), stream_ptr()),
          "dr_emb_pool_bwd_sorted")


def emb_pool_bwd_dups_apply(ids, row_base, plan, D, num_rows, grad, d_fm_logit, scale, dst_table, dst_lin, dst_bias, sum_x, x_sorted,
                            lin_old_t, table_amax, wg_workspace, wg_R, wg_scale, dstW, dstb=None, wg_h2=True, parts=1):
    ids = _c(ids, torch.int64)
    B, F = ids.shape
    wg_F, wg_N = dstW.shape
    assert grad.stride(1) == 1 and dstW.stride(1) == 1
    assert lin_old_t is None or (lin_old_t.shape == (F, B) and lin_old_t.is_contiguous() and lin_old_t.dtype == torch.float32)
    check(lib().dr_emb_pool_bwd_dups_apply(ptr(ids), ptr(row_base), ptr(plan.rows), ptr(plan.slots), ptr(plan.flags), ptr(plan.dup_heads),
                                           ptr(plan.dup_count), B, F, D, int(num_rows), ptr(grad), grad.stride(0), ptr(sum_x),
                                           ptr(d_fm_logit), float(scale), ptr(dst_table), ptr(dst_lin), ptr(dst_bias), ptr(x_sorted),
                                           ptr(lin_old_t), int(parts) | 8, ptr(table_amax), ptr(wg_workspace), wg_workspace.numel() * 4,
                                           int(wg_R), wg_F, wg_N, 1 if wg_h2 else 0, float(wg_scale), ptr(dstW), dstW.stride(0), ptr(dstb),
                                           stream_ptr()), "dr_emb_pool_bwd_dups_apply")


def h2_dgrad_emb_sgd(dy, dy_amax, w: "H2Planes", ids_t, plan, row_base, table, lin_w, lin_old_t, sum_x, d_fm_logit, scale, d_concat,
                     table_amax=None):
    F, M = ids_t.shape
    K = dy.shape[1]
    assert dy.stride(1) == 1 and d_concat.stride(1) == 1 and table.is_contiguous() and table.shape[1] == 64 and sum_x.is_contiguous()
    assert ids_t.dtype == torch.int32 and ids_t.is_contiguous() and dy.shape[0] == M and w.rows >= 64 * F
    assert (lin_w is None) == (lin_old_t is None)
    assert lin_old_t is None or (lin_old_t.shape == (F, M) and lin_old_t.is_contiguous())
    check(lib().dr_h2_dgrad_emb_sgd(ptr(dy), dy.stride(0), ptr(dy_amax), ptr(w.buf), w.plane_stride, w.ld, ptr(w.amax), M, F, K,
                                    ptr(ids_t), ptr(plan.flags), ptr(row_base), ptr(table), ptr(lin_w), ptr(lin_old_t), ptr(sum_x),
                                    ptr(d_fm_logit), float(scale), ptr(d_concat), d_concat.stride(0), ptr(table_amax), stream_ptr()),
          "dr_h2_dgrad_emb_sgd")


def emb_lin_update_unique(ids, row_base, plan, d_fm_logit, scale, dst_lin, slot_lin_grad=None):
    ids = _c(ids, torch.int64)
    B, F = ids.shape
    check(lib().dr_emb_lin_update_unique(ptr(ids), ptr(plan.flags), B, F, ptr(row_base), ptr(d_fm_logit), ptr(slot_lin_grad),
                                         float(scale), ptr(dst_lin), stream_ptr()), "dr_emb_lin_update_unique")


def adam_lr_t(lr, beta1, beta2, step):
    return lr * (1.0 - beta2 ** step) ** 0.5 / (1.0 - beta1 ** step)


def emb_pool_bwd_sorted_adam(ids, row_base, plan, D, num_rows, grad, d_fm_logit, lr_t, beta1, beta2, eps, table, m_table,
                             v_table, lin_w=None, m_lin=None, v_lin=None, concat=None, sum_x=None, slot_lin_grad=None, x_sorted=None,
                             lin_old_t=None, table_amax=None):
    ids = _c(ids, torch.int64)
    B, F = ids.shape
    assert grad.stride(1) == 1
    assert lin_old_t is None or (lin_old_t.shape == (F, B) and lin_old_t.is_contiguous())
    check(lib().dr_emb_pool_bwd_sorted_adam(ptr(ids), ptr(row_base), ptr(plan.rows), ptr(plan.slots), ptr(plan.flags),
                                            ptr(plan.dup_heads), ptr(plan.dup_count), B, F, D, int(num_rows), ptr(grad),
                                            grad.stride(0), ptr(concat), concat.stride(0) if concat is not None else 0,
                                            ptr(sum_x), ptr(d_fm_logit), ptr(slot_lin_grad), float(lr_t), float(beta1),
                                            float(beta2), float(eps), ptr(table), ptr(m_table), ptr(v_table), ptr(lin_w),
                                            ptr(m_lin), ptr(v_lin), ptr(x_sorted), ptr(lin_old_t), ptr(table_amax), stream_ptr()),
          "dr_emb_pool_bwd_sorted_adam")


def adam_catchup_rows(ids, row_base, table, m_table, v_table, lin_w, m_lin, v_lin, row_step, upto, stamp, lr, beta1=0.9,
                      beta2=0.999, eps=1e-8):
    ids = _c(ids, torch.int64)
    B, F = ids.shape
    assert row_step.dtype == torch.int32 and row_step.is_contiguous()
    check(lib().dr_adam_catchup_rows(ptr(ids), B * F, F, ptr(row_base), table.shape[1], ptr(table), ptr(m_table), ptr(v_table),
                                     ptr(lin_w), ptr(m_lin), ptr(v_lin), ptr(row_step), int(upto), int(stamp), float(lr),
                                     float(beta1), float(beta2), float(eps), stream_ptr()), "dr_adam_catchup_rows")


def adam_step(param, grad, m, v, lr_t, beta1=0.9, beta2=0.999, eps=1e-8, grad_scale=1.0):
    assert param.is_contiguous() and grad.is_contiguous() and m.is_contiguous() and v.is_contiguous()
    n = param.numel()
    assert grad.numel() == n and m.numel() == n and v.numel() == n
    check(lib().dr_adam_step(ptr(param), ptr(grad), ptr(m), ptr(v), n, float(lr_t), float(beta1), float(beta2), float(eps),
                             float(grad_scale), stream_ptr()), "dr_adam_step")


def ftrl_step(param, grad, accum, linear, lr, lr_power=-0.5, l1=0.0, l2=0.0, grad_scale=1.0):
    assert param.is_contiguous() and grad.is_contiguous() and accum.is_contiguous() and linear.is_contiguous()
    n = param.numel()
    assert grad.numel() == n and accum.numel() == n and linear.numel() == n
    check(lib().dr_ftrl_step(ptr(param), ptr(grad), ptr(accum), ptr(linear), n, float(lr), float(lr_power), float(l1), float(l2),
                             float(grad_scale), stream_ptr()), "dr_ftrl_step")


def linear_bwd_dx_fm(dy, W, d_fm_logit, sum_x, concat, D, FD, out):
    dy = _rowmajor_ld4(dy)
    W = _rowmajor_ld4(W)
    M, N = dy.shape
    K = W.shape[0]
    check(lib().dr_linear_bwd_dx_fm(ptr(dy), dy.stride(0), ptr(W), W.stride(0), M, K, N, ptr(d_fm_logit), ptr(sum_x),
                                    ptr(concat), concat.stride(0), int(D), int(FD), ptr(out), out.stride(0),
                                    stream_ptr()), "dr_linear_bwd_dx_fm")
# ... 596 lines not shown
    assert lin_vals_t is None or (lin_vals_t.shape == (F, M) and lin_vals_t.is_contiguous() and lin_vals_t.dtype == torch.float32)
    check(lib().dr_h2_emb_linear_fwd(ptr(ids), M, F, ptr(row_base), int(field_rows_max), ptr(table), table.shape[1], ptr(table_amax), ptr(lin_w),
                                     ptr(lin_bias), ptr(dense_pad), ptr(dense_amax), ptr(concat), concat.stride(0) if concat is not None else 0,
                                     int(K), ptr(wt.buf), wt.plane_stride, wt.ld, ptr(wt.amax), wt.rows, ptr(bias), int(act), ptr(sum_x),
                                     ptr(fm_logit), ptr(out), out.stride(0), ptr(lin_vals_t), stream_ptr()), "dr_h2_emb_linear_fwd")
    return out


def h2_emb_linear_tail_supported(M, N, H):
    return N == 256 and 0 < H <= 32 and M > 0 and M % 32 == 0


def h2_emb_linear_tail_workspace(M, device):
    return torch.empty(max(128, lib().dr_h2_emb_linear_tail_fwd_workspace_bytes(int(M)) // 4), dtype=torch.float32, device=device)


def h2_emb_linear_tail_fwd(ids, row_base, field_rows_max, table, table_amax, lin_w, lin_bias, dense_pad, dense_amax, concat, K, wt: H2Planes, bias,
                           act, sum_x, fm_logit, out, W1, b1, W2, b2, labels, loss_mode, scale, dx, lin_vals_t=None, dst_W1="inplace",
                           dst_b1="inplace", dst_W2="inplace", dst_b2="inplace", prob=None, d_logit=None, d_h=None, loss=None, workspace=None,
                           parts=3, dx_amax=None):
    ids = _c(ids, torch.int64)
    M, F = ids.shape
    N, H = wt.rows, W1.shape[1]
    dev = table.device
    dst_W1 = W1 if isinstance(dst_W1, str) else dst_W1
    dst_b1 = b1 if isinstance(dst_b1, str) else dst_b1
    dst_W2 = W2 if isinstance(dst_W2, str) else dst_W2
    dst_b2 = b2 if isinstance(dst_b2, str) else dst_b2
    assert (concat is None or concat.stride(1) == 1) and wt.cols == K and (out is None or (out.stride(1) == 1 and out.shape == (M, N)))
    assert dense_pad is None or (dense_pad.shape == (M, 32) and dense_pad.is_contiguous())
    assert lin_vals_t is None or (lin_vals_t.shape == (F, M) and lin_vals_t.is_contiguous() and lin_vals_t.dtype == torch.float32)
    assert W1.shape[0] == N and W1.stride(1) == 1 and dst_W1.stride(1) == 1 and W2.shape == (H, 1) and dx.shape == (M, N) and dx.stride(1) == 1
    assert labels.numel() == M and labels.is_contiguous() and labels.dtype == torch.float32
    prob = prob if prob is not None else torch.empty(M, dtype=torch.float32, device=dev)
    d_logit = d_logit if d_logit is not None else torch.empty(M, dtype=torch.float32, device=dev)
    loss = loss if loss is not None else torch.empty(1, dtype=torch.float32, device=dev)
    if workspace is None:
        workspace = h2_emb_linear_tail_workspace(M, dev)
    check(lib().dr_h2_emb_linear_tail_fwd(
        ptr(ids), M, F, ptr(row_base), int(field_rows_max), ptr(table), table.shape[1], ptr(table_amax), ptr(lin_w), ptr(lin_bias),
        ptr(dense_pad), ptr(dense_amax), ptr(concat), concat.stride(0) if concat is not None else 0, int(K), ptr(wt.buf), wt.plane_stride,
        wt.ld, ptr(wt.amax), N, ptr(bias), int(act), ptr(sum_x), ptr(fm_logit), ptr(out), out.stride(0) if out is not None else 0,
        ptr(lin_vals_t), ptr(W1), W1.stride(0), ptr(b1), H, ptr(W2), W2.stride(0), ptr(b2), ptr(labels), int(loss_mode), float(scale),
        ptr(dst_W1), dst_W1.stride(0), ptr(dst_b1), ptr(dst_W2), dst_W2.stride(0) if dst_W2 is not None else 0, ptr(dst_b2), ptr(prob),
        ptr(d_logit), ptr(d_h), d_h.stride(0) if d_h is not None else 0, ptr(dx), dx.stride(0), ptr(loss), ptr(workspace),
        workspace.numel() * 4, int(parts), ptr(dx_amax), stream_ptr()), "dr_h2_emb_linear_tail_fwd")
    return loss, prob, d_logit, dx


def h2_wgrad(x, x_amax, dy, dy_amax, scale, dstW, dstb=None, workspace=None):
    R, F = x.shape
    N = dy.shape[1]
    assert x.stride(1) == 1 and dy.stride(1) == 1 and dstW.shape == (F, N) and dstW.stride(1) == 1 and dy.shape[0] == R
    if workspace is None:
        workspace = bf3_wgrad_workspace(R, F, N, x.device)
    check(lib().dr_h2_wgrad(ptr(x), x.stride(0), ptr(x_amax), ptr(dy), dy.stride(0), ptr(dy_amax), R, F, N, float(scale), ptr(dstW),
                            dstW.stride(0), ptr(dstb), ptr(workspace), workspace.numel() * 4, stream_ptr()), "dr_h2_wgrad")
    return dstW


def h2_wgrad_emb(ids_t, row_base, table, table_amax, dense_pad, dense_amax, dy, dy_amax, scale, dstW, dstb=None, workspace=None, parts=3):
    nf, R = ids_t.shape
    F, N = dstW.shape
    assert ids_t.dtype == torch.int32 and ids_t.is_contiguous() and dy.stride(1) == 1 and dstW.stride(1) == 1 and dy.shape == (R, N)
    assert dense_pad is None or (dense_pad.shape == (R, 32) and dense_pad.is_contiguous())
    if workspace is None:
        workspace = bf3_wgrad_workspace(R, F, N, dy.device)
    check(lib().dr_h2_wgrad_emb(ptr(ids_t), R, nf, ptr(row_base), ptr(table), table.shape[1], ptr(table_amax), ptr(dense_pad), ptr(dense_amax),
                                ptr(dy), dy.stride(0), ptr(dy_amax), F, N, float(scale), ptr(dstW), dstW.stride(0), ptr(dstb), ptr(workspace),
                                workspace.numel() * 4, int(parts), stream_ptr()), "dr_h2_wgrad_emb")
    return dstW


class H2WeightPlanes:

    def __init__(self, W, double_buffer=False):
        K, N = W.shape
        self.W = W
        self.amax = h2_record(W.device)
        self.wt = H2Planes(N, K, W.device, self.amax)
        self.w = H2Planes(K, N, W.device, self.amax)
        self._w_alt = H2Planes(K, N, W.device, h2_record(W.device)) if double_buffer else None
        self._parts = None
        self.refresh()

    def refresh(self):
        if self._parts is None:
            self._parts = torch.zeros(256, dtype=torch.int32, device=self.W.device)
        K, N = self.W.shape
        if self._w_alt is not None:
            self.w, self._w_alt = self._w_alt, self.w
            self.amax = self.w.amax
            self.wt.amax = self.amax
        check(lib().dr_h2_refresh_weight(ptr(self.W), self.W.stride(0), K, N, ptr(self.w.buf), self.w.plane_stride, self.w.ld,
                                         ptr(self.wt.buf), self.wt.plane_stride, self.wt.ld, ptr(self.amax), ptr(self._parts),
                                         stream_ptr()), "dr_h2_refresh_weight")
        self._ver = self.W._version

    def ensure_fresh(self):
        if self.W._version != self._ver:
            self.refresh()


def planes_worthwhile(M, K, N):
    return get_gemm_mode() == "bf16x3" and M >= 2048 and N >= 128 and K >= 64


def bf3_gemm_tn_workspace(R, F, N, device):
    return torch.empty(max(64, lib().dr_bf3_gemm_tn_workspace_bytes(int(R), int(F), int(N)) // 4), dtype=torch.float32,
                       device=device)


def bf3_gemm_tn(x: Planes, y: Planes, scale, dstW, y_colsum=None, dstb=None, workspace=None):
    R, F, N = x.rows, x.cols, y.cols
    assert y.rows == R and dstW.shape == (F, N) and dstW.stride(1) == 1
    if workspace is None:
        workspace = bf3_gemm_tn_workspace(R, F, N, x.buf.device)
    check(lib().dr_bf3_gemm_tn(ptr(x.buf), x.plane_stride, x.ld, ptr(y.buf), y.plane_stride, y.ld, R, F, N, float(scale),
                               ptr(dstW), dstW.stride(0), ptr(y_colsum), ptr(dstb), ptr(workspace), workspace.numel() * 4,
                               stream_ptr()), "dr_bf3_gemm_tn")
    return dstW


ACT_CODES = {None: 0, "linear": 0, "relu": 1, "sigmoid": 2, "tanh": 3}


def cin_fwd(x0, x, W, bias=None, act=2):
    x0, x, W = _c(x0, torch.float32), _c(x, torch.float32), _c(W, torch.float32)
    B, H0, D = x0.shape
    Hk = x.shape[1]
    Fm = W.shape[1]
    if x.shape != (B, Hk, D) or W.shape[0] != H0 * Hk:
        raise ValueError("cin_fwd: shapes do not agree (x0 %s, x %s, W %s)" % (tuple(x0.shape), tuple(x.shape), tuple(W.shape)))
    bias = _dense_arg(bias, "cin_fwd: bias", numel=Fm)
    out = torch.empty((B, Fm, D), dtype=torch.float32, device=x0.device)
    check(lib().dr_cin_fwd(ptr(x0), ptr(x), B, H0, Hk, D, ptr(W), Fm, ptr(bias), int(act), ptr(out), stream_ptr()), "dr_cin_fwd")
    return out


def cin_bwd(x0, x, W, act, out, d_out, want_bias=False):
    x0, x, W, d_out = _c(x0, torch.float32), _c(x, torch.float32), _c(W, torch.float32), _c(d_out, torch.float32)
    B, H0, D = x0.shape
    Hk, Fm = x.shape[1], W.shape[1]
    if x.shape != (B, Hk, D) or W.shape[0] != H0 * Hk:
        raise ValueError("cin_bwd: shapes do not agree (x0 %s, x %s, W %s)" % (tuple(x0.shape), tuple(x.shape), tuple(W.shape)))
    out = _dense_arg(out, "cin_bwd: out", shape=(B, Fm, D))
    d_out = _dense_arg(d_out, "cin_bwd: d_out", shape=(B, Fm, D))
    d_x0, d_x, dW = torch.empty_like(x0), torch.empty_like(x), torch.empty_like(W)
    dbias = torch.empty(Fm, dtype=torch.float32, device=x0.device) if want_bias else None
    check(lib().dr_cin_bwd(ptr(x0), ptr(x), B, H0, Hk, D, ptr(W), Fm, int(act), ptr(out), ptr(d_out), ptr(d_x0), ptr(d_x), ptr(dW),
                           ptr(dbias), stream_ptr()), "dr_cin_bwd")
    return d_x0, d_x, dW, dbias


def _cin_pool_dims(x0, x, W):
    if x0.dim() != 3 or x.dim() != 3 or W.dim() != 2:
        raise ValueError("cin_pool: x0 [B, H0, D], x [B, Hk, D], W [H0 * Hk, Fm] (got %s, %s, %s)"
                         % (tuple(x0.shape), tuple(x.shape), tuple(W.shape)))
    B, H0, D = x0.shape
    Hk, Fm = x.shape[1], W.shape[1]
    if x.shape != (B, Hk, D) or W.shape[0] != H0 * Hk:
        raise ValueError("cin_pool: shapes do not agree (x0 %s, x %s, W %s)" % (tuple(x0.shape), tuple(x.shape), tuple(W.shape)))
    return B, H0, Hk, D, Fm


def cin_pool_fwd(x0, x, W, bias=None, act=0, want_out=True, want_pooled=True):
    x0, x, W = _c(x0, torch.float32), _c(x, torch.float32), _c(W, torch.float32)
    B, H0, Hk, D, Fm = _cin_pool_dims(x0, x, W)
    out = torch.empty((B, Fm, D), dtype=torch.float32, device=x0.device) if want_out else None
    pooled = torch.empty((B, Fm), dtype=torch.float32, device=x0.device) if want_pooled else None
    check(lib().dr_cin_pool_fwd(ptr(x0), ptr(x), B, H0, Hk, D, ptr(W), Fm, ptr(None if bias is None else _c(bias, torch.float32)), int(act),
                                ptr(out), ptr(pooled), stream_ptr()), "dr_cin_pool_fwd")
    return out, pooled


def cin_pool_bwd_partials(B, H0, Hk, D, Fm):
# ... 1383 lines not shown
```

include/dr_hotpath.h:

```cpp
#ifndef DR_HOTPATH_H
#define DR_HOTPATH_H

#include <stdint.h>

#ifdef __cplusplus
extern "C" {
#endif

#define DR_OK 0
#define DR_EINVAL (-1)
#define DR_ELAUNCH (-2)
#define DR_ESHAPE (-3)

typedef void* dr_stream_t;

const char* dr_version(void);

#define DR_GEMM_BF16X3 0
#define DR_GEMM_NATIVE_F32 1
int32_t dr_set_gemm_mode(int32_t mode);
int32_t dr_get_gemm_mode(void);

#define DR_GEMM_SPLIT_BF16X3 0
#define DR_GEMM_SPLIT_F16X2 1
int32_t dr_set_gemm_split(int32_t split);
int32_t dr_get_gemm_split(void);

int dr_hash_bucket_i64(const int64_t* keys, int64_t B, int32_t C, const uint64_t* col_buckets,
                       int64_t* ids_out, dr_stream_t stream);

int dr_ids_transpose_i32(const int64_t* ids, int64_t B, int32_t F, int32_t* out, dr_stream_t stream);
int dr_hash_bucket_bytes(const uint8_t* bytes, const int64_t* offsets, int64_t n,
                         uint64_t num_buckets, int64_t* ids_out, dr_stream_t stream);

int dr_vocab_lookup_i64(const int64_t* keys, int64_t n, const int64_t* vocab, int32_t vocab_len,
                        int64_t* ids_out, dr_stream_t stream);
int dr_vocab_lookup_bytes(const uint8_t* bytes, const int64_t* offsets, int64_t n,
                          const uint8_t* vocab_bytes, const int64_t* vocab_offsets,
                          int32_t vocab_len, int64_t* ids_out, dr_stream_t stream);

#define DR_POOL_FIRST_ORDER_ONLY 1
int dr_emb_pool_fwd(const int64_t* ids, int64_t B, int32_t F, int32_t C, const int32_t* col_start,
                    const int64_t* row_base, const float* table, int32_t D,
                    const float* lin_w, const float* lin_bias,
                    float* concat, int64_t ld_concat, float* sum_x, float* fm_logit,
                    int32_t flags, dr_stream_t stream);
int dr_lin_fields_fwd(const int64_t* ids, int64_t B, int32_t F, int32_t C, const int32_t* col_start,
                      const int64_t* row_base, const float* lin_w, float* out, int64_t ld_out,
                      dr_stream_t stream);
int dr_lin_fields_bwd(const int64_t* ids, int64_t B, int32_t F, int32_t C, const int32_t* col_start,
                      const int64_t* row_base, const float* d_out, int64_t ld_dout, float scale,
                      float* dst_lin, dr_stream_t stream);


int dr_emb_pool_bwd(const int64_t* ids, int64_t B, int32_t F, int32_t C, const int32_t* col_start,
                    const int64_t* row_base, int32_t D,
                    const float* d_concat, int64_t ld_dconcat,
                    const float* concat, int64_t ld_concat, const float* sum_x,
                    const float* d_fm_logit, float scale,
                    float* dst_table, float* dst_lin, float* dst_bias, dr_stream_t stream);

int64_t dr_emb_sort_workspace_bytes(int64_t n);
int32_t dr_emb_plan_set_small_limit(int32_t limit);
int dr_emb_sort_slots(const int64_t* ids, int64_t B, int32_t F, const int64_t* row_base, int64_t num_rows,
                      int64_t* sorted_rows, int32_t* sorted_slots, uint8_t* unique_flags,
                      int32_t* dup_heads, int32_t* dup_count, void* workspace, int64_t workspace_bytes,
                      dr_stream_t stream);
int dr_hash_sort_slots(const int64_t* keys, int64_t B, int32_t F, const uint64_t* col_buckets, int64_t* ids_out,
                       int32_t* ids_t_out, const int64_t* row_base, int64_t num_rows, int64_t* sorted_rows,
                       int32_t* sorted_slots, uint8_t* unique_flags, int32_t* dup_heads, int32_t* dup_count, void* workspace,
                       int64_t workspace_bytes, dr_stream_t stream);
int dr_emb_pool_bwd_sorted(const int64_t* ids, const int64_t* row_base, const int64_t* sorted_rows,
                           const int32_t* sorted_slots, const uint8_t* unique_flags,
                           const int32_t* dup_heads, const int32_t* dup_count, int64_t B, int32_t F,
                           int32_t D, int64_t num_rows, const float* grad, int64_t ld_grad,
                           const float* concat, int64_t ld_concat, const float* sum_x,
                           const float* d_fm_logit, const float* slot_lin_grad, float scale,
                           float* dst_table, float* dst_lin, float* dst_bias, float* x_sorted,
                           const float* lin_old_t, int32_t parts, uint32_t* table_amax, dr_stream_t stream);
int dr_emb_lin_update_unique(const int64_t* ids, const uint8_t* unique_flags, int64_t B, int32_t F, const int64_t* row_base,
                             const float* d_fm_logit, const float* slot_lin_grad, float scale, float* dst_lin, dr_stream_t stream);
int dr_emb_snapshot_sorted_rows(const int64_t* sorted_rows, const int32_t* dup_heads, const int32_t* dup_count,
                                const float* table, int32_t D, int64_t num_rows, float* x_sorted, dr_stream_t stream);

int dr_emb_pool_bwd_sorted_adam(const int64_t* ids, const int64_t* row_base, const int64_t* sorted_rows,
                                const int32_t* sorted_slots, const uint8_t* unique_flags,
                                const int32_t* dup_heads, const int32_t* dup_count, int64_t B, int32_t F,
                                int32_t D, int64_t num_rows, const float* grad, int64_t ld_grad,
                                const float* concat, int64_t ld_concat, const float* sum_x,
                                const float* d_fm_logit, const float* slot_lin_grad, float lr_t, float beta1,
                                float beta2, float eps, float* table, float* m_table, float* v_table,
                                float* lin_w, float* m_lin, float* v_lin, float* x_sorted, const float* lin_old_t,
                                uint32_t* table_amax, dr_stream_t stream);
int dr_adam_catchup_rows(const int64_t* ids, int64_t n, int32_t F, const int64_t* row_base, int32_t D, float* table,
                         float* m_table, float* v_table, float* lin_w, float* m_lin, float* v_lin, int32_t* row_step,
                         int32_t upto, int32_t stamp, float lr, float beta1, float beta2, float eps, dr_stream_t stream);
int dr_adam_step(float* param, const float* grad, float* m, float* v, int64_t n, float lr_t, float beta1,
                 float beta2, float eps, float grad_scale, dr_stream_t stream);

int dr_ftrl_step(float* param, const float* grad, float* accum, float* linear, int64_t n, float lr,
                 float lr_power, float l1, float l2, float grad_scale, dr_stream_t stream);



int dr_fm2_fwd(const float* x, int64_t B, int32_t F, int32_t D, float* out, dr_stream_t stream);
int dr_fm2_bwd(const float* x, const float* d_out, int64_t B, int32_t F, int32_t D, float* dx,
               dr_stream_t stream);

int dr_linear_fwd(const float* x, int64_t ld_x, const float* W, int64_t ld_w, const float* b,
                  int64_t M, int32_t K, int32_t N, int32_t act, float* y, int64_t ld_y,
                  dr_stream_t stream);
int dr_linear_bwd_dx(const float* dy, int64_t ld_dy, const float* W, int64_t ld_w, int64_t M,
                     int32_t K, int32_t N, const float* relu_src, int64_t ld_relu_src,
                     int32_t accumulate, float* dx, int64_t ld_dx, dr_stream_t stream);
int64_t dr_linear_fwd_splitk_workspace_bytes(int64_t M, int32_t K, int32_t N);
int dr_linear_fwd_splitk(const float* x, int64_t ld_x, const float* W, int64_t ld_w, int64_t M, int32_t K, int32_t N,
                         float* y, int64_t ld_y, float* workspace, int64_t workspace_bytes, dr_stream_t stream);

int dr_linear_bwd_dx_fm(const float* dy, int64_t ld_dy, const float* W, int64_t ld_w, int64_t M,
                        int32_t K, int32_t N, const float* d_fm_logit, const float* sum_x,
                        const float* concat, int64_t ld_concat, int32_t D, int32_t FD, float* dx,
                        int64_t ld_dx, dr_stream_t stream);
int64_t dr_linear_bwd_dw_workspace_bytes(int64_t M, int32_t K, int32_t N);
int dr_linear_bwd_dw(const float* x, int64_t ld_x, const float* dy, int64_t ld_dy, int64_t M,
                     int32_t K, int32_t N, float scale, float* dstW, int64_t ld_w, float* dstb,
                     float* workspace, int64_t workspace_bytes, dr_stream_t stream);
int64_t dr_linear_bwd_narrow_workspace_bytes(int64_t M, int32_t K, int32_t N);
int dr_linear_bwd_narrow(const float* x, int64_t ld_x, const float* dy, int64_t ld_dy, const float* W,
                         int64_t ld_w, int64_t M, int32_t K, int32_t N, int32_t relu_mask, float scale,
                         float* dstW, int64_t ld_dstw, float* dstb, float* dx, int64_t ld_dx,
                         void* workspace, int64_t workspace_bytes, int32_t parts, uint32_t* dx_amax, dr_stream_t stream);

int64_t dr_tower_head_workspace_bytes(int64_t M);
int dr_tower_head_fwd_bwd(const float* x, int64_t ld_x, const float* W1, int64_t ld_w1, const float* b1,
                          int64_t M, int64_t n_total, int32_t K, int32_t H, int32_t act, const float* w2,
                          int64_t ld_w2, const float* b2, const float* extra_logit, const float* labels,
                          int32_t loss_mode, float scale, float* dst_w2, int64_t ld_dst_w2, float* dst_b2, float* h_out, int64_t ld_h,
                          float* prob, float* d_logit, float* d_h, int64_t ld_dh, float* loss_out, void* workspace,
                          int64_t workspace_bytes, int32_t parts, dr_stream_t stream);
int64_t dr_tower_tail_workspace_bytes(int64_t M, int32_t K);
int dr_tower_tail_fused(const float* x, int64_t ld_x, const float* W1, int64_t ld_w1, const float* b1, int64_t M, int64_t n_total,
                        int32_t K, int32_t H, const float* w2, int64_t ld_w2, const float* b2, const float* extra_logit,
                        const float* labels, int32_t loss_mode, float scale, float* dst_w1, int64_t ld_dst_w1, float* dst_b1,
                        float* dst_w2, int64_t ld_dst_w2, float* dst_b2, float* prob, float* d_logit, float* d_h, int64_t ld_dh,
                        float* dx, int64_t ld_dx, float* loss_out, void* workspace, int64_t workspace_bytes, int32_t parts,
                        uint32_t* dx_amax, dr_stream_t stream);


int dr_cross_fwd(const float* x0, const float* x, int64_t ld, const float* W, int64_t ld_w,
                 const float* b, float diag_scale, int64_t M, int32_t Dm, float* out,
                 float* prod_out, dr_stream_t stream);
int dr_cross_combine_bwd(const float* x0, const float* prod, const float* d_out, int64_t M,
                         int32_t Dm, int64_t ld, float diag_scale, float* d_prod, float* d_x0_accum,
                         float* d_x_accum, uint32_t* d_prod_amax, dr_stream_t stream);
// ... 86 lines not shown
                 dr_stream_t stream);
int dr_bf3_join(const void* planes, int64_t plane_stride, int64_t ld_planes, int64_t R, int32_t C, float* dst,
                int64_t ld_dst, dr_stream_t stream);
int dr_bf3_gemm_nt(const void* a_planes, int64_t a_plane_stride, int64_t a_ld, const void* b_planes,
                   int64_t b_plane_stride, int64_t b_ld, int64_t M, int32_t N, int32_t K, const float* bias,
                   int32_t act, const float* mask, int64_t ld_mask, float* C, int64_t ldc, dr_stream_t stream);
int dr_bf3_linear_nt(const float* A, int64_t lda, const void* b_planes, int64_t b_plane_stride, int64_t b_ld, int64_t M,
                     int32_t N, int32_t K, const float* bias, int32_t act, const float* mask, int64_t ld_mask,
                     int32_t accumulate, float* C, int64_t ldc, dr_stream_t stream);
int dr_bf3_linear_nt_pack(const float* dy, int64_t ld_dy, const void* w_planes, int64_t plane_stride, int64_t b_ld, int64_t M,
                          int32_t N, int32_t K, const int64_t* pos, int32_t F, const float* d_fm_logit, const float* sum_x,
                          const float* x, int64_t ld_x, float* out_rows, float* out_lin, float* bias_sum, dr_stream_t stream);
int dr_h2_linear_nt_pack(const float* dy, int64_t ld_dy, const uint32_t* dy_amax, const void* w_planes, int64_t plane_stride,
                         int64_t b_ld, const uint32_t* w_amax, int64_t M, int32_t N, int32_t K, const int64_t* pos, int32_t F,
                         const float* d_fm_logit, const float* sum_x, const float* x, int64_t ld_x, float* out_rows,
                         float* out_lin, float* bias_sum, dr_stream_t stream);
int dr_bf3_cross_fwd(const float* x0, const float* x, int64_t ld, const void* wt_planes, int64_t plane_stride,
                     int64_t ld_planes, const float* b, float diag_scale, int64_t M, int32_t Dm, float* out,
                     float* prod_out, dr_stream_t stream);
int dr_bf3_emb_linear_fwd(const int64_t* ids, int64_t M, int32_t F, const int64_t* row_base, int64_t field_rows_max,
                          const float* table, int32_t D, const float* lin_w, const float* lin_bias, const float* dense_pad, float* concat,
                          int64_t ld_concat, int32_t K, const void* wt_planes, int64_t plane_stride, int64_t ld_planes, int32_t N,
                          const float* bias, int32_t act, float* sum_x, float* fm_logit, float* out, int64_t ld_out,
                          float* lin_vals_t, dr_stream_t stream);
int64_t dr_bf3_wgrad_workspace_bytes(int64_t R, int32_t F, int32_t N);
int dr_bf3_wgrad(const float* x, int64_t ld_x, const float* dy, int64_t ld_dy, int64_t R, int32_t F, int32_t N,
                 float scale, float* dstW, int64_t ld_w, float* dstb, void* workspace, int64_t workspace_bytes,
                 dr_stream_t stream);
int dr_bf3_wgrad_emb(const int32_t* ids_t, int64_t R, int32_t nf, const int64_t* row_base, const float* table, int32_t D,
                     const float* dense_pad, const float* dy, int64_t ld_dy, int32_t F, int32_t N, float scale, float* dstW,
                     int64_t ld_w, float* dstb, void* workspace, int64_t workspace_bytes, int32_t parts, dr_stream_t stream);
int64_t dr_bf3_gemm_tn_workspace_bytes(int64_t R, int32_t F, int32_t N);
int dr_bf3_gemm_tn(const void* x_planes, int64_t x_plane_stride, int64_t x_ld, const void* y_planes,
                   int64_t y_plane_stride, int64_t y_ld, int64_t R, int32_t F, int32_t N, float scale, float* dst,
                   int64_t ld_dst, const float* y_colsum, float* dstb, void* workspace, int64_t workspace_bytes,
                   dr_stream_t stream);

int dr_h2_amax(const float* src, int64_t ld, int64_t R, int32_t C, uint32_t* amax, int32_t reset, dr_stream_t stream);
int dr_h2_split(const float* src, int64_t ld_src, int64_t R, int32_t C, void* planes, int64_t plane_stride, int64_t ld_planes,
                int64_t row_offset, int64_t col_offset, int32_t transpose, const uint32_t* amax, dr_stream_t stream);
int dr_h2_refresh_weight(const float* W, int64_t ldw, int64_t K, int32_t N, void* w_planes, int64_t w_plane_stride, int64_t w_ld,
                         void* wt_planes, int64_t wt_plane_stride, int64_t wt_ld, uint32_t* amax, uint32_t* parts, dr_stream_t stream);
int dr_h2_linear_nt(const float* A, int64_t lda, const uint32_t* a_amax, const void* b_planes, int64_t b_plane_stride, int64_t b_ld,
                    const uint32_t* b_amax, int64_t M, int32_t N, int32_t K, const float* bias, int32_t act, const float* mask,
                    int64_t ld_mask, int32_t accumulate, float* C, int64_t ldc, uint32_t* c_amax, dr_stream_t stream);
int dr_h2_dgrad_emb_sgd(const float* dy, int64_t ld_dy, const uint32_t* dy_amax, const void* w_planes, int64_t w_plane_stride,
                        int64_t w_ld, const uint32_t* w_amax, int64_t M, int32_t F, int32_t K, const int32_t* ids_t,
                        const uint8_t* unique_flags, const int64_t* row_base, float* table, float* lin_w, const float* lin_old_t,
                        const float* sum_x, const float* d_fm_logit, float scale, float* d_concat, int64_t ld_dconcat,
                        uint32_t* table_amax, dr_stream_t stream);
int dr_h2_cross_fwd(const float* x0, const float* x, int64_t ld, const uint32_t* x_amax, const void* wt_planes, int64_t plane_stride,
                    int64_t ld_planes, const uint32_t* w_amax, const float* b, float diag_scale, int64_t M, int32_t Dm, float* out,
                    float* prod_out, uint32_t* out_amax, dr_stream_t stream);
int dr_h2_emb_linear_fwd(const int64_t* ids, int64_t M, int32_t F, const int64_t* row_base, int64_t field_rows_max, const float* table,
                         int32_t D, const uint32_t* table_amax, const float* lin_w, const float* lin_bias, const float* dense_pad,
                         const uint32_t* dense_amax, float* concat, int64_t ld_concat, int32_t K, const void* wt_planes,
                         int64_t plane_stride, int64_t ld_planes, const uint32_t* w_amax, int32_t N, const float* bias, int32_t act,
                         float* sum_x, float* fm_logit, float* out, int64_t ld_out, float* lin_vals_t, dr_stream_t stream);
int64_t dr_h2_emb_linear_tail_fwd_workspace_bytes(int64_t M);
int dr_h2_emb_linear_tail_fwd(const int64_t* ids, int64_t M, int32_t F, const int64_t* row_base, int64_t field_rows_max,
                              const float* table, int32_t D, const uint32_t* table_amax, const float* lin_w, const float* lin_bias,
                              const float* dense_pad, const uint32_t* dense_amax, float* concat, int64_t ld_concat, int32_t K,
                              const void* wt_planes, int64_t plane_stride, int64_t ld_planes, const uint32_t* w_amax, int32_t N,
                              const float* bias, int32_t act, float* sum_x, float* fm_logit, float* out, int64_t ld_out,
                              float* lin_vals_t, const float* W1, int64_t ld_w1, const float* b1, int32_t H, const float* w2,
                              int64_t ld_w2, const float* b2, const float* labels, int32_t loss_mode, float scale, float* dst_w1,
                              int64_t ld_dst_w1, float* dst_b1, float* dst_w2, int64_t ld_dst_w2, float* dst_b2, float* prob,
                              float* d_logit, float* d_h, int64_t ld_dh, float* dx, int64_t ld_dx, float* loss_out, void* workspace,
                              int64_t workspace_bytes, int32_t parts, uint32_t* dx_amax, dr_stream_t stream);
int dr_h2_wgrad(const float* x, int64_t ld_x, const uint32_t* x_amax, const float* dy, int64_t ld_dy, const uint32_t* dy_amax, int64_t R,
                int32_t F, int32_t N, float scale, float* dstW, int64_t ld_w, float* dstb, void* workspace, int64_t workspace_bytes,
                dr_stream_t stream);
int dr_h2_wgrad_emb(const int32_t* ids_t, int64_t R, int32_t nf, const int64_t* row_base, const float* table, int32_t D,
                    const uint32_t* table_amax, const float* dense_pad, const uint32_t* dense_amax, const float* dy, int64_t ld_dy,
                    const uint32_t* dy_amax, int32_t F, int32_t N, float scale, float* dstW, int64_t ld_w, float* dstb, void* workspace,
                    int64_t workspace_bytes, int32_t parts, dr_stream_t stream);
int dr_emb_pool_bwd_dups_apply(const int64_t* ids, const int64_t* row_base, const int64_t* sorted_rows, const int32_t* sorted_slots,
                               const uint8_t* unique_flags, const int32_t* dup_heads, const int32_t* dup_count, int64_t B, int32_t F,
                               int32_t D, int64_t num_rows, const float* grad, int64_t ld_grad, const float* sum_x,
                               const float* d_fm_logit, float scale, float* dst_table, float* dst_lin, float* dst_bias, float* x_sorted,
                               const float* lin_old_t, int32_t parts, uint32_t* table_amax, void* wg_workspace,
                               int64_t wg_workspace_bytes, int64_t wg_R, int32_t wg_F, int32_t wg_N, int32_t wg_h2, float wg_scale,
                               float* dstW, int64_t ld_w, float* dstb, dr_stream_t stream);


int dr_cin_fwd(const float* x0, const float* x, int64_t B, int32_t H0, int32_t Hk, int32_t D, const float* W,
               int32_t Fm, const float* bias, int32_t act, float* out, dr_stream_t stream);
int dr_cin_bwd(const float* x0, const float* x, int64_t B, int32_t H0, int32_t Hk, int32_t D, const float* W,
               int32_t Fm, int32_t act, const float* out, const float* d_out, float* d_x0, float* d_x, float* dW,
               float* dbias, dr_stream_t stream);

int dr_cin_pool_fwd(const float* x0, const float* x, int64_t B, int32_t H0, int32_t Hk, int32_t D, const float* W, int32_t Fm,
                    const float* bias, int32_t act, float* out, float* pooled, dr_stream_t stream);
int64_t dr_cin_pool_bwd_workspace_bytes(int64_t B, int32_t H0, int32_t Hk, int32_t D, int32_t Fm);
int dr_cin_pool_bwd(const float* x0, const float* x, int64_t B, int32_t H0, int32_t Hk, int32_t D, const float* W, int32_t Fm,
                    int32_t act, const float* out, const float* d_out, const float* d_pooled, float* d_x0, int32_t accumulate_x0,
                    float* d_x, float* dW, float* dbias, void* ws, int64_t ws_bytes, dr_stream_t stream);

int dr_dot_interact_fwd(const float* dense, int64_t ld_dense, const float* emb, int64_t ld_emb, int64_t B, int32_t F, int32_t D,
                        int32_t self_interaction, float* out, int64_t ld_out, dr_stream_t stream);
int dr_dot_interact_bwd(const float* dense, int64_t ld_dense, const float* emb, int64_t ld_emb, const float* d_out, int64_t ld_dout,
                        int64_t B, int32_t F, int32_t D, int32_t self_interaction, float* d_dense, int64_t ld_ddense, float* d_emb,
                        int64_t ld_demb, dr_stream_t stream);

int dr_afm_pool_fwd(const float* emb, int64_t ld_emb, const float* W, const float* b, const float* h, int64_t B, int32_t F, int32_t D,
                    int32_t A, float* out, int64_t ld_out, float* lse, float* attn, int64_t ld_attn, dr_stream_t stream);
int64_t dr_afm_pool_bwd_workspace_bytes(int64_t B, int32_t F, int32_t D, int32_t A);
int dr_afm_pool_bwd(const float* emb, int64_t ld_emb, const float* W, const float* b, const float* h, const float* out, int64_t ld_out,
                    const float* lse, const float* d_out, int64_t ld_dout, int64_t B, int32_t F, int32_t D, int32_t A, float* d_emb,
                    int64_t ld_demb, float* dW, float* db, float* dh, void* ws, int64_t ws_bytes, dr_stream_t stream);

int dr_gru_seq_fwd(const float* xp, int64_t ld_xp, const float* U, const float* h0, const int32_t* lengths, const float* att, int64_t B,
                   int32_t T, int32_t H, float* hs, int64_t ld_hs, float* h_last, dr_stream_t stream);
int64_t dr_gru_seq_bwd_workspace_bytes(int64_t B, int32_t T, int32_t H);
int dr_gru_seq_bwd(const float* xp, int64_t ld_xp, const float* U, const float* h0, const int32_t* lengths, const float* att,
                   const float* hs, int64_t ld_hs, int64_t B, int32_t T, int32_t H, const float* d_hs, int64_t ld_dhs,
                   const float* d_h_last, float* d_xp, int64_t ld_dxp, float* dU, float* d_h0, float* d_att, void* ws, int64_t ws_bytes,
                   dr_stream_t stream);
int dr_seq_attn_fwd(const float* hs, int64_t ld_hs, const float* q, const int32_t* lengths, int64_t B, int32_t T, int32_t H, float* a,
                    dr_stream_t stream);
int dr_seq_attn_bwd(const float* hs, int64_t ld_hs, const float* q, const int32_t* lengths, const float* a, const float* d_a, int64_t B,
                    int32_t T, int32_t H, float* d_hs, int64_t ld_dhs, float* d_q, dr_stream_t stream);

int dr_ffm_fwd(const float* rows, int64_t ld_rows, int64_t B, int32_t F, int32_t k, float* inter, dr_stream_t stream);
int dr_ffm_bwd(const float* rows, int64_t ld_rows, const float* d_inter, int64_t B, int32_t F, int32_t k, float* d_rows, int64_t ld_d,
               dr_stream_t stream);
int dr_ffm_gather_fwd(const int64_t* ids, int64_t B, int32_t F, const int64_t* row_base, const float* table, int32_t k,
                      const float* lin_w, const float* lin_bias, float* inter, float* first_order, dr_stream_t stream);
int dr_ffm_gather_bwd(const int64_t* ids, int64_t B, int32_t F, const int64_t* row_base, const float* table, int32_t k,
                      const float* d_inter, float* d_rows, int64_t ld_d, dr_stream_t stream);

#define DR_SGNS_SKIP_EQUAL 1
int dr_sgns_fwd(const float* in_table, const float* out_table, int32_t D, const int64_t* centers, const int64_t* contexts,
                const int64_t* negatives, int64_t B, int32_t K, const float* sample_weight, int32_t flags, float row_scale,
                float* loss_rows, float* coeff, float* scores, float* d_center, int64_t ld_dc, float* d_ctx, int64_t ld_dx,
                dr_stream_t stream);
int dr_sgns_bwd(const float* in_table, const float* out_table, int32_t D, const int64_t* centers, const int64_t* contexts,
                const int64_t* negatives, int64_t B, int32_t K, int32_t flags, const float* coeff, const float* d_loss, float* d_center,
                int64_t ld_dc, float* d_ctx, int64_t ld_dx, dr_stream_t stream);

int dr_alias_sample(const float* prob, const int32_t* alias, int64_t V, int64_t n, uint64_t seed, uint64_t offset, int64_t* out,
                    dr_stream_t stream);
int dr_random_walk(const int64_t* row_ptr, const int32_t* col, int64_t n_rows, const int64_t* starts, int64_t W, int32_t L,
                   uint64_t seed, int64_t* walks, dr_stream_t stream);
int dr_random_walk_weighted(const int64_t* row_ptr, const int32_t* col, const int64_t* cum, int64_t n_rows, const int64_t* starts,
                            int64_t W, int32_t L, uint64_t seed, int64_t* walks, dr_stream_t stream);

int dr_eges_fwd(const float* side_table, int32_t D, const int64_t* row_base, const int64_t* side_ids, int32_t S, const float* att,
                int64_t ld_att, const int64_t* att_ids, const float* out_table, const int64_t* contexts, int32_t P,
                const int64_t* negatives, int32_t K, int64_t B, const float* sample_weight, int32_t flags, float row_scale,
                float* loss_rows, float* coeff, float* alpha, float* scores, float* d_side, int64_t ld_ds, float* d_att, int64_t ld_da,
                float* d_ctx, int64_t ld_dx, dr_stream_t stream);
int dr_eges_bwd(const float* side_table, int32_t D, const int64_t* row_base, const int64_t* side_ids, int32_t S, const float* att,
                const int64_t* att_ids, const float* out_table, const int64_t* contexts, int32_t P, const int64_t* negatives, int32_t K,
                int64_t B, int32_t flags, const float* coeff, const float* alpha, const float* d_loss, float* d_side, int64_t ld_ds,
                float* d_att, int64_t ld_da, float* d_ctx, int64_t ld_dx, dr_stream_t stream);
int dr_eges_embed(const float* side_table, int32_t D, const int64_t* row_base, const int64_t* side_ids, int32_t S, const float* att,
                  int64_t ld_att, const int64_t* att_ids, int64_t n, float* out, int64_t ld_out, dr_stream_t stream);

int dr_pnn_outer_fwd(const float* emb, int64_t ld_emb, const float* W, int64_t ld_w, const float* addend, int64_t ld_add, int64_t B,
                     int32_t F, int32_t D, int32_t N, float* u, int64_t ld_u, float* out, int64_t ld_out, dr_stream_t stream);
int64_t dr_pnn_outer_bwd_workspace_bytes(int64_t B, int32_t F, int32_t D, int32_t N);
int dr_pnn_outer_bwd(const float* u, int64_t ld_u, const float* W, int64_t ld_w, const float* d_out, int64_t ld_dout, int64_t B,
                     int32_t F, int32_t D, int32_t N, float* d_emb, int64_t ld_demb, int32_t accumulate, float* dW, int64_t ld_dw,
                     void* ws, int64_t ws_bytes, dr_stream_t stream);

// ... 108 lines not shown
```

Measured before the change: 72.51 million examples/sec.

## Fuse h2 weight-plane refresh into embedding backward apply kernels as riders

The wgrad reduce riders in the duplicate-apply kernel now also emit per-block amax partials. The hot-rows apply kernel gains extra blocks that split the updated weight into f16x2 planes, replacing a separate amax-plus-refresh launch pair. Hash/sort is also split into front and back parts so the two halves can be scheduled separately. This removes kernel launches and a dependency bubble, but shares grids between unrelated work and adds an extra API path.

```diff
diff --git a/deep_recommenders_amd/csrc/bf3_planes.hip b/deep_recommenders_amd/csrc/bf3_planes.hip
--- a/deep_recommenders_amd/csrc/bf3_planes.hip
+++ b/deep_recommenders_amd/csrc/bf3_planes.hip
@@ -1,4 +1,5 @@
 #include "bf3_rs_core.h"
+#include "tn_rs_reduce.h"
 
 namespace {
 
@@ -556,29 +557,8 @@
                                                             _Float16* __restrict__ w, int64_t w_ps, int64_t w_ld,
                                                             _Float16* __restrict__ wt, int64_t wt_ps, int64_t wt_ld,
                                                             const uint32_t* __restrict__ parts, int32_t nparts, uint32_t* __restrict__ amax) {
-    uint32_t m = (int)threadIdx.x < nparts ? parts[threadIdx.x] : 0u;
-#pragma unroll
-    for (int o = 32; o > 0; o >>= 1) m = max(m, (uint32_t)__shfl_xor((int)m, o, 64));
-    __shared__ uint32_t wm[4];
-    if ((threadIdx.x & 63) == 0) wm[threadIdx.x >> 6] = m;
-    __syncthreads();
-    m = max(max(wm[0], wm[1]), max(wm[2], wm[3]));
-    if (blockIdx.x == 0 && threadIdx.x == 0) amax[0] = m;
-    float sc, inv;
-    h2_scale_of(m, sc, inv);
-    h2_mode_on();
-    const int64_t total = R * (int64_t)C, stride = (int64_t)gridDim.x * blockDim.x;
-    for (int64_t i = (int64_t)blockIdx.x * blockDim.x + threadIdx.x; i < 2 * total; i += stride) {
-        int64_t r, c, off;
-        _Float16* dst;
-        int64_t ps;
-        if (i < total) { r = i / C; c = i - r * C; off = r * w_ld + c; dst = w; ps = w_ps; }
-        else { const int64_t j = i - total; c = j / R; r = j - c * R; off = c * wt_ld + r; dst = wt; ps = wt_ps; }
-        const float v = src[r * ld + c] * sc;
-        const _Float16 h = (_Float16)v;
-        dst[off] = h;
-        dst[ps + off] = (_Float16)(v - (float)h);
-    }
+    h2_split_both_block(H2RefreshRide{src, ld, R, C, w, w_ps, w_ld, wt, wt_ps, wt_ld, parts, nparts, amax},
+                        (int)blockIdx.x, (int)gridDim.x, (int)threadIdx.x);
 }
 
 __global__ __launch_bounds__(256) void bf3_join_kernel(const __bf16* __restrict__ planes, int64_t ps, int64_t ldp, int64_t R,
diff --git a/deep_recommenders_amd/csrc/emb_plan.hip b/deep_recommenders_amd/csrc/emb_plan.hip
--- a/deep_recommenders_amd/csrc/emb_plan.hip
+++ b/deep_recommenders_amd/csrc/emb_plan.hip
@@ -573,7 +573,7 @@
 namespace {
 int plan_small_front(const int64_t* raw, const uint64_t* col_buckets, int64_t* ids_out, int32_t* ids_t, const int64_t* ids, int64_t B,
                      int32_t F, const int64_t* row_base, int64_t num_rows, uint64_t* rows_y, uint64_t* keys_x, uint32_t* ghist,
-                     uint32_t* tot, Ctrl* ctrl, int32_t* dup_count, hipStream_t s) {
+                     uint32_t* tot, Ctrl* ctrl, int32_t* dup_count, hipStream_t s, int parts) {
     const int64_t n64 = B * F;
     const int32_t n = (int32_t)n64;
     const uint32_t mul = (uint32_t)((((uint64_t)RADIX) << 32) / (uint64_t)num_rows);
@@ -585,17 +585,18 @@
     if (chunk > 0x7fffffff) return DR_EINVAL;
     const bool trans = ids_t != nullptr;
     const size_t lds = (size_t)8 * (raw ? 3 : 1) * F + (trans ? (size_t)4 * 64 * (F + 1) : 0);
-    if (raw) {
+    if (raw && (parts & 1)) {
         if (trans)
             hipLaunchKernelGGL((plan_front_kernel<true, true>), dim3(nbf), dim3(256), lds, s, raw, B, F, col_buckets, ids_out, ids_t, row_base,
                                (uint64_t)num_rows, mul, (int32_t)sub, rows_y, ghist);
         else
             hipLaunchKernelGGL((plan_front_kernel<true, false>), dim3(nbf), dim3(256), lds, s, raw, B, F, col_buckets, ids_out, ids_t,
                                row_base, (uint64_t)num_rows, mul, (int32_t)sub, rows_y, ghist);
-    } else {
+    } else if (!raw && (parts & 2)) {
         hipLaunchKernelGGL((plan_front_kernel<false, false>), dim3(nbf), dim3(256), lds, s, ids, B, F, col_buckets, ids_out, ids_t, row_base,
                            (uint64_t)num_rows, mul, (int32_t)sub, rows_y, ghist);
     }
+    if (!(parts & 2)) return DR_OK;
     hipLaunchKernelGGL((radix_scan_kernel<true>), dim3(RADIX), dim3(256), 0, s, ghist, (int32_t)nbf, tot, ctrl, dup_count);
     hipLaunchKernelGGL(plan_scatter_kernel, dim3(nbs), dim3(LG_T), 0, s, rows_y, keys_x, n, mul, (int32_t)chunk, ghist, (int32_t)nbf, tot);
     return DR_OK;
@@ -603,7 +604,8 @@
 
 int sort_slots_impl(const int64_t* raw, const uint64_t* col_buckets, int32_t* ids_t, const int64_t* ids, int64_t B, int32_t F,
                     const int64_t* row_base, int64_t num_rows, int64_t* sorted_rows, int32_t* sorted_slots, uint8_t* unique_flags,
-                    int32_t* dup_heads, int32_t* dup_count, void* workspace, int64_t workspace_bytes, dr_stream_t stream) {
+                    int32_t* dup_heads, int32_t* dup_count, void* workspace, int64_t workspace_bytes, dr_stream_t stream,
+                    int parts = 3) {
     if (B < 0 || F <= 0 || num_rows <= 0) return DR_EINVAL;
     const int64_t n64 = B * F;
     if (n64 == 0) return DR_OK;
@@ -628,15 +630,19 @@
 
     const bool claimable = n64 <= (1 << 24) && num_rows < 0x7fffffffLL;
     const bool fused_front = raw != nullptr && claimable && F <= 64;
-    if (raw && !fused_front) {
+    if (raw && !fused_front && (parts & 1)) {
         int rc = dr_hash_bucket_i64(raw, B, F, col_buckets, const_cast<int64_t*>(ids), stream);
         if (rc == DR_OK && ids_t) rc = dr_ids_transpose_i32(ids, B, F, ids_t, stream);
         if (rc != DR_OK) return rc;
     }
     if (claimable) {
         int rc = plan_small_front(fused_front ? raw : nullptr, col_buckets, const_cast<int64_t*>(ids), fused_front ? ids_t : nullptr, ids, B,
-                                  F, row_base, num_rows, rows_y, keys_x, ghist, tot, ctrl, dup_count, s);
+                                  F, row_base, num_rows, rows_y, keys_x, ghist, tot, ctrl, dup_count, s, parts);
         if (rc != DR_OK) return rc;
+        if (!(parts & 2)) {
+            DR_CHECK_LAUNCH();
+            return DR_OK;
+        }
         static const hipError_t lds_optin = hipFuncSetAttribute(reinterpret_cast<const void*>(plan_lds_claim_kernel),
                                                                 hipFuncAttributeMaxDynamicSharedMemorySize, 4 << LDS_TAB_MAX_LOG);
         if (lds_optin != hipSuccess) return DR_ELAUNCH;
@@ -651,6 +657,7 @@
         DR_CHECK_LAUNCH();
         return DR_OK;
     }
+    if (!(parts & 2)) return DR_OK;
     if (hipMemsetAsync(dup_count, 0, 2 * sizeof(int32_t), s) != hipSuccess) return DR_ELAUNCH;
     const unsigned bits = bits_for((uint64_t)num_rows);
     const int passes = (int)((bits + RADIX_BITS - 1) / RADIX_BITS);
@@ -690,3 +697,12 @@
     return sort_slots_impl(keys, col_buckets, ids_t_out, ids_out, B, F, row_base, num_rows, sorted_rows, sorted_slots, unique_flags,
                            dup_heads, dup_count, workspace, workspace_bytes, stream);
 }
+
+extern "C" int dr_hash_sort_slots_parts(const int64_t* keys, int64_t B, int32_t F, const uint64_t* col_buckets, int64_t* ids_out,
+                                        int32_t* ids_t_out, const int64_t* row_base, int64_t num_rows, int64_t* sorted_rows,
+                                        int32_t* sorted_slots, uint8_t* unique_flags, int32_t* dup_heads, int32_t* dup_count,
+                                        void* workspace, int64_t workspace_bytes, int32_t parts, dr_stream_t stream) {
+    if (!keys || !col_buckets || !ids_out || parts < 1 || parts > 3) return DR_EINVAL;
+    return sort_slots_impl(keys, col_buckets, ids_t_out, ids_out, B, F, row_base, num_rows, sorted_rows, sorted_slots, unique_flags,
+                           dup_heads, dup_count, workspace, workspace_bytes, stream, parts);
+}
diff --git a/deep_recommenders_amd/csrc/emb_sorted.hip b/deep_recommenders_amd/csrc/emb_sorted.hip
--- a/deep_recommenders_amd/csrc/emb_sorted.hip
+++ b/deep_recommenders_amd/csrc/emb_sorted.hip
@@ -348,7 +348,8 @@
 }
 
 template <int LPR>
-__global__ __launch_bounds__(256) void emb_bwd_dups_apply_kernel(BwdSortedArgs a, drrs::TnRsApply ap, int grid_d) {
+__global__ __launch_bounds__(256) void emb_bwd_dups_apply_kernel(BwdSortedArgs a, drrs::TnRsApply ap, int grid_d,
+                                                                 uint32_t* __restrict__ amax_parts) {
     const int bid = blockIdx.x;
     if (bid < grid_d)
         emb_bwd_dups_body<LPR, false>(bid, grid_d, a.rows, a.slots, a.n, a.dup_heads, a.dup_count, a.F, a.D, a.num_rows, a.grad, a.ld,
@@ -356,19 +357,30 @@
                                       a.det != 0, a.amax);
     else if (bid == grid_d) {
         if (a.lin_bias != nullptr && a.d_fm_logit != nullptr) dr_block_sum_axpy(a.d_fm_logit, a.B, a.scale, a.lin_bias);
-    } else
-        drrs::tn_rs_reduce_ride(ap, bid - grid_d - 1, (int)gridDim.x - grid_d - 1, threadIdx.x);
+    } else {
+        const int rider = bid - grid_d - 1;
+        uint32_t m = drrs::tn_rs_reduce_ride(ap, rider, (int)gridDim.x - grid_d - 1, threadIdx.x);
+        if (amax_parts != nullptr) {
+            __shared__ uint32_t wm[4];
+            m = drrs::block_max_256(m, wm, threadIdx.x);
+            if (threadIdx.x == 0) amax_parts[rider] = m;
+        }
+    }
 }
 
 template <int LPR>
-__global__ __launch_bounds__(256) void emb_bwd_hot_apply_kernel(BwdSortedArgs a) {
+__global__ __launch_bounds__(256) void emb_bwd_hot_apply_kernel(BwdSortedArgs a, drrs::H2RefreshRide rf, int grid_h) {
+    if ((int)blockIdx.x >= grid_h) {
+        drrs::h2_split_both_block(rf, (int)blockIdx.x - grid_h, (int)gridDim.x - grid_h, threadIdx.x);
+        return;
+    }
     constexpr int NS = DR_WAVE / LPR;
     const int lane = threadIdx.x & 63, grp = lane / LPR, sub = lane % LPR;
     const int D = a.D, F = a.F;
     const bool dvalid = sub < (D >> 2);
     const int subc = dvalid ? sub : (D >> 2) - 1;
     const bool any_lin = a.lin_w != nullptr && (a.d_fm_logit != nullptr || a.slot_lin != nullptr);
-    const int64_t nwaves = (int64_t)gridDim.x * (blockDim.x >> 6);
+    const int64_t nwaves = (int64_t)grid_h * (blockDim.x >> 6);
     const int64_t wave0 = (int64_t)blockIdx.x * (blockDim.x >> 6) + (threadIdx.x >> 6);
     const int64_t nheads = a.dup_count[0], n = a.dup_count[1];
     float wmax = 0.f;
@@ -465,7 +477,8 @@
                            int64_t ld_grad, const float* concat, int64_t ld_concat, const float* sum_x,
                            const float* d_fm_logit, const float* slot_lin_grad, float scale, float* dst_table,
                            float* dst_lin, float* dst_bias, const AdamArgs* adam, float* x_sorted, dr_stream_t stream,
-                           int parts, const float* lin_old_t, uint32_t* table_amax, const drrs::TnRsApply* apply = nullptr) {
+                           int parts, const float* lin_old_t, uint32_t* table_amax, const drrs::TnRsApply* apply = nullptr,
+                           const drrs::H2RefreshRide* refresh = nullptr) {
     if (B < 0 || F <= 0 || F > 64 || D < 4 || D > 256 || (D & 3) || num_rows <= 0) return DR_EINVAL;
     const int64_t n = B * F;
     if (n == 0) return DR_OK;
@@ -495,10 +508,11 @@
     constexpr int K4_U_OVERRIDE = 0;
 #endif
     const int nlb = apply != nullptr ? drrs::tn_rs_reduce_blocks(apply->F, apply->N, apply->vec) : 0;
-    const int riders = nlb < 1024 ? nlb : 1024;
+    const int riders = nlb < drrs::H2_REFRESH_MAX_PARTS ? nlb : drrs::H2_REFRESH_MAX_PARTS;
 #define LAUNCH(L, ADAM_)                                                                                              \
     { if (apply != nullptr) {                                                                                         \
-        hipLaunchKernelGGL((emb_bwd_dups_apply_kernel<L>), dim3(grid_d + 1 + riders), dim3(256), 0, dr_s(stream), ba, *apply, grid_d);     \
+        hipLaunchKernelGGL((emb_bwd_dups_apply_kernel<L>), dim3(grid_d + 1 + riders), dim3(256), 0, dr_s(stream), ba, *apply, grid_d,      \
+                           refresh != nullptr ? const_cast<uint32_t*>(refresh->parts) : nullptr);                     \
     } else {                                                                                                          \
         constexpr int NS_ = 64 / L;                                                                                   \
         constexpr int U_ = K4_U_OVERRIDE > 0 ? K4_U_OVERRIDE : (NS_ >= 16 ? 2 : 4);                                   \
@@ -521,8 +535,16 @@
 #undef CALL
 #undef LAUNCH
     DR_CHECK_LAUNCH();
-    if (det && (parts & 2)) {
-#define HOT(L) hipLaunchKernelGGL((emb_bwd_hot_apply_kernel<L>), dim3(1024), dim3(256), 0, dr_s(stream), ba)
+    if ((det || refresh != nullptr) && (parts & 2)) {
+        const int grid_h = det ? 1024 : 0;
+        drrs::H2RefreshRide rf{};
+        int riders_s = 0;
+        if (refresh != nullptr) {
+            rf = *refresh;
+            rf.nparts = riders;
+            riders_s = dr_grid_for(2 * rf.R * (int64_t)rf.C, 256, 2048);
+        }
+#define HOT(L) hipLaunchKernelGGL((emb_bwd_hot_apply_kernel<L>), dim3(grid_h + riders_s), dim3(256), 0, dr_s(stream), ba, rf, grid_h)
         switch (lpr) {
             case 1: HOT(1); break;
             case 2: HOT(2); break;
@@ -561,6 +583,26 @@
                                           int32_t wg_N, int32_t wg_h2, float wg_scale, float* dstW, int64_t ld_w, float* dstb,
                                           dr_stream_t stream) {
     if (parts != 9 && parts != 11) return DR_EINVAL;
+    return dr_emb_pool_bwd_dups_apply_refresh(ids, row_base, sorted_rows, sorted_slots, unique_flags, dup_heads, dup_count, B, F, D, num_rows,
+                                              grad, ld_grad, sum_x, d_fm_logit, scale, dst_table, dst_lin, dst_bias, x_sorted, lin_old_t, parts,
+                                              table_amax, wg_workspace, wg_workspace_bytes, wg_R, wg_F, wg_N, wg_h2, wg_scale, dstW, ld_w, dstb,
+                                              nullptr, 0, 0, nullptr, 0, 0, nullptr, nullptr, stream);
+}
+
+extern "C" int dr_emb_pool_bwd_dups_apply_refresh(const int64_t* ids, const int64_t* row_base, const int64_t* sorted_rows,
+                                                  const int32_t* sorted_slots, const uint8_t* unique_flags, const int32_t* dup_heads,
+                                                  const int32_t* dup_count, int64_t B, int32_t F, int32_t D, int64_t num_rows,
+                                                  const float* grad, int64_t ld_grad, const float* sum_x, const float* d_fm_logit, float scale,
+                                                  float* dst_table, float* dst_lin, float* dst_bias, float* x_sorted, const float* lin_old_t,
+                                                  int32_t parts, uint32_t* table_amax, void* wg_workspace, int64_t wg_workspace_bytes,
+                                                  int64_t wg_R, int32_t wg_F, int32_t wg_N, int32_t wg_h2, float wg_scale, float* dstW,
+                                                  int64_t ld_w, float* dstb, void* w_planes, int64_t w_plane_stride, int64_t w_ld,
+                                                  void* wt_planes, int64_t wt_plane_stride, int64_t wt_ld, uint32_t* w_amax,
+                                                  uint32_t* amax_parts, dr_stream_t stream) {
+    if (parts != 9 && parts != 11 && !(parts == 10 && w_planes != nullptr)) return DR_EINVAL;
+    if (w_planes != nullptr && (!wt_planes || !w_amax || !amax_parts || w_ld < wg_N || wt_ld < wg_F || w_plane_stride <= 0 ||
+                                wt_plane_stride <= 0))
+        return DR_EINVAL;
     if (wg_R <= 0 || wg_F <= 0 || wg_N <= 0 || !wg_workspace || !dstW || ld_w < wg_N) return DR_EINVAL;
     if (wg_workspace_bytes < dr_bf3_wgrad_workspace_bytes(wg_R, wg_F, wg_N)) return DR_EINVAL;
     if (B <= 0) return DR_EINVAL;
@@ -568,9 +610,11 @@
     int64_t per;
     drrs::tn_rs_plan(wg_R, wg_F, wg_N, split, per, Fp, Np);
     const drrs::TnRsApply ap = drrs::tn_rs_apply_of(wg_workspace, split, wg_F, wg_N, Fp, Np, wg_h2 != 0, wg_scale, dstW, ld_w, dstb);
+    const drrs::H2RefreshRide rf{dstW, ld_w, wg_F, wg_N, static_cast<_Float16*>(w_planes), w_plane_stride, w_ld,
+                                 static_cast<_Float16*>(wt_planes), wt_plane_stride, wt_ld, amax_parts, 0, w_amax};
     return bwd_sorted_impl(ids, row_base, sorted_rows, sorted_slots, unique_flags, dup_heads, dup_count, B, F, D, num_rows, grad, ld_grad,
                            nullptr, 0, sum_x, d_fm_logit, nullptr, scale, dst_table, dst_lin, dst_bias, nullptr, x_sorted, stream, parts,
-                           lin_old_t, table_amax, &ap);
+                           lin_old_t, table_amax, &ap, w_planes != nullptr ? &rf : nullptr);
 }
 
 namespace {
diff --git a/deep_recommenders_amd/csrc/tn_rs_reduce.h b/deep_recommenders_amd/csrc/tn_rs_reduce.h
--- a/deep_recommenders_amd/csrc/tn_rs_reduce.h
+++ b/deep_recommenders_amd/csrc/tn_rs_reduce.h
@@ -21,13 +21,13 @@
 }
 
 template <int V>
-__device__ __forceinline__ void tn_rs_reduce_block(const TnRsApply& a, int lb, int tid) {
+__device__ __forceinline__ uint32_t tn_rs_reduce_block(const TnRsApply& a, int lb, int tid) {
     typedef float vec_t __attribute__((ext_vector_type(V)));
     const int w = (a.N + V - 1) / V;
     const int64_t t = (int64_t)lb * TN_RS_RED_THREADS + tid;
     const int f = (int)(t / w);
     const int n = (int)(t - (int64_t)f * w) * V;
-    if (f >= a.F) return;
+    if (f >= a.F) return 0u;
     const int split = a.split, N = a.N, Np = a.Np;
     const int64_t ps = (int64_t)a.Fp * Np;
     float wscale = a.scale;
@@ -52,15 +52,22 @@
     };
     const vec_t acc = sum_slices(a.partial + (int64_t)f * Np + n, ps);
     float* d = a.dst + (int64_t)f * a.ld + n;
+    uint32_t wmax = 0u;
     if (V == 1 || n + V <= N) {
         vec_t o = *reinterpret_cast<vec_t*>(d);
 #pragma unroll
-        for (int c = 0; c < V; ++c) o[c] = fmaf(wscale, acc[c], o[c]);
+        for (int c = 0; c < V; ++c) {
+            o[c] = fmaf(wscale, acc[c], o[c]);
+            wmax = max(wmax, __float_as_uint(fabsf(o[c])));
+        }
         *reinterpret_cast<vec_t*>(d) = o;
     } else {
 #pragma unroll
         for (int c = 0; c < V; ++c)
-            if (n + c < N) d[c] = fmaf(wscale, acc[c], d[c]);
+            if (n + c < N) {
+                d[c] = fmaf(wscale, acc[c], d[c]);
+                wmax = max(wmax, __float_as_uint(fabsf(d[c])));
+            }
     }
     if (f == 0 && a.colsum != nullptr && a.dstb != nullptr) {
         const vec_t cacc = sum_slices(a.colsum + n, Np);
@@ -68,13 +75,56 @@
         for (int c = 0; c < V; ++c)
             if (n + c < N) a.dstb[n + c] = fmaf(a.scale, cacc[c], a.dstb[n + c]);
     }
+    return wmax;
 }
 
-__device__ __forceinline__ void tn_rs_reduce_ride(const TnRsApply& a, int rider, int nriders, int tid) {
+__device__ __forceinline__ uint32_t tn_rs_reduce_ride(const TnRsApply& a, int rider, int nriders, int tid) {
     const int nlb = tn_rs_reduce_blocks(a.F, a.N, a.vec);
-    for (int lb = rider; lb < nlb; lb += nriders) {
-        if (a.vec) tn_rs_reduce_block<4>(a, lb, tid);
-        else tn_rs_reduce_block<1>(a, lb, tid);
+    uint32_t wmax = 0u;
+    for (int lb = rider; lb < nlb; lb += nriders)
+        wmax = max(wmax, a.vec ? tn_rs_reduce_block<4>(a, lb, tid) : tn_rs_reduce_block<1>(a, lb, tid));
+    return wmax;
+}
+
+__device__ __forceinline__ uint32_t block_max_256(uint32_t m, uint32_t* wm, int tid) {
+#pragma unroll
+    for (int o = 32; o > 0; o >>= 1) m = max(m, (uint32_t)__shfl_xor((int)m, o, 64));
+    if ((tid & 63) == 0) wm[tid >> 6] = m;
+    __syncthreads();
+    return max(max(wm[0], wm[1]), max(wm[2], wm[3]));
+}
+
+struct H2RefreshRide {
+    const float* src; int64_t ld; int64_t R; int32_t C;
+    _Float16* w; int64_t w_ps, w_ld;
+    _Float16* wt; int64_t wt_ps, wt_ld;
+    const uint32_t* parts; int32_t nparts;
+    uint32_t* amax;
+};
+constexpr int H2_REFRESH_MAX_PARTS = 1024;
+
+__device__ __forceinline__ void h2_split_both_block(const H2RefreshRide& r, int blk, int nblk, int tid) {
+    uint32_t m = 0u;
+    for (int p = tid; p < r.nparts; p += 256) m = max(m, r.parts[p]);
+    __shared__ uint32_t wm[4];
+    m = block_max_256(m, wm, tid);
+    if (blk == 0 && tid == 0) r.amax[0] = m;
+    float sc, inv;
+    h2_scale_of(m, sc, inv);
+    h2_mode_on();
+    const int64_t R = r.R;
+    const int32_t C = r.C;
+    const int64_t total = R * (int64_t)C, stride = (int64_t)nblk * 256;
+    for (int64_t i = (int64_t)blk * 256 + tid; i < 2 * total; i += stride) {
+        int64_t rr, c, off;
+        _Float16* dst;
+        int64_t ps;
+        if (i < total) { rr = i / C; c = i - rr * C; off = rr * r.w_ld + c; dst = r.w; ps = r.w_ps; }
+        else { const int64_t j = i - total; c = j / R; rr = j - c * R; off = c * r.wt_ld + rr; dst = r.wt; ps = r.wt_ps; }
+        const float v = r.src[rr * r.ld + c] * sc;
+        const _Float16 h = (_Float16)v;
+        dst[off] = h;
+        dst[ps + off] = (_Float16)(v - (float)h);
     }
 }
 
diff --git a/deep_recommenders_amd/engine.py b/deep_recommenders_amd/engine.py
--- a/deep_recommenders_amd/engine.py
+++ b/deep_recommenders_amd/engine.py
@@ -192,8 +192,11 @@
         self.overlap_dw = _ov == "1"
         if self.overlap_dw:
             self.no_concat = False
-        self.fold_reduces = (os.environ.get("DR_FOLD_REDUCES", "1") != "0" and self.tail_in_fwd and self.fuse_k4 and self.h2
+        _fr = os.environ.get("DR_FOLD_REDUCES", "2")
+        self.fold_reduces = (_fr != "0" and self.tail_in_fwd and self.fuse_k4 and self.h2
                              and optimizer == "sgd" and not self.overlap_dw and not self.reduce_side)
+        self.fold_planes = self.fold_reduces and _fr != "1"
+        self.ids_event_early = os.environ.get("DR_IDS_EVENT", "1") != "0"
         self.concurrent = {}
         if self.overlap_dw:
             k4 = "emb_pool_bwd_adam" if optimizer == "adam" else "emb_pool_bwd"
@@ -299,10 +302,18 @@
                 self._ev_dense[nxt].record(self.side_r)
         with torch.cuda.stream(self.side):
             self.side.wait_event(self.ev_fwd0)
+            def chain(parts):
+                ops.hash_sort_slots(nk, self.col_buckets, self.row_base, self.R, self._ids[nxt],
+                                    self._ids_t[nxt] if self.no_concat else None, self._plans[nxt], parts=parts)
+
+            def chain_in_parts():
+                chain(1)
+                self._ev_hashed[nxt].record(self.side)
+                chain(2)
             self._k("next_batch: hash_sort_slots(side stream, overlapped)", "overlap", self.B * self.F * 52,
-                    lambda: ops.hash_sort_slots(nk, self.col_buckets, self.row_base, self.R, self._ids[nxt],
-                                                self._ids_t[nxt] if self.no_concat else None, self._plans[nxt]))
-            self._ev_hashed[nxt].record(self.side)
+                    chain_in_parts if self.ids_event_early else (lambda: chain(3)))
+            if not self.ids_event_early:
+                self._ev_hashed[nxt].record(self.side)
             self._ev_sorted[nxt].record(self.side)
         self._early_issued = True
 
@@ -659,7 +670,8 @@
 
     def _backward_l0_fused_k4(self, x, dy, sc, dstW, dstb, fl):
         lr = self.lr
-        torch.cuda.current_stream().wait_event(self.ev_sorted)
+        if not self.ids_event_early:
+            torch.cuda.current_stream().wait_event(self.ev_sorted)
         fold = self.fold_reduces
         self._k("linear_bwd_dw_L0", "mfma", fl, lambda: self._wgrad(0, x, dy, sc, dstW, dstb, main_only=fold))
         w_old = self.wplanes[0].w
@@ -681,6 +693,8 @@
         mark = self._prefetch_mark()
         if early:
             self._prefetch_issue(mark)
+        if self.ids_event_early:
+            torch.cuda.current_stream().wait_event(self.ev_sorted)
         if not self._k4_det:
             ops.emb_snapshot_sorted_rows(self.plan, self.table, self.R, self.x_sorted)
         work = self.alg_bytes_bwd() - 4.0 * self.B * self.F * self.D + 4.0 * self.B * dy.shape[1]
@@ -691,14 +705,18 @@
                                                    self.table, self.lin_w, self.lin_bias, sum_x=self.sum_x, x_sorted=self.x_sorted,
                                                    parts=parts | 8, lin_old_t=self.lin_old_t, table_amax=self.tab_amax)
         if fold:
-            self._k("emb_pool_bwd_dups", "hbm", 0,
-                    lambda: ops.emb_pool_bwd_dups_apply(self.ids, self.row_base, self.plan, self.D, self.R, self.d_concat, self.d_logit, -lr,
-                                                        self.table, self.lin_w, self.lin_bias, self.sum_x, self.x_sorted, self.lin_old_t,
-                                                        self.tab_amax, self.wg_ws[0], self.B, sc, dstW, dstb, wg_h2=True, parts=1))
-            refresh_planes_behind()
+            tgt = self.wplanes[0].hand_off() if self.fold_planes else None
+            dups = lambda parts: ops.emb_pool_bwd_dups_apply(self.ids, self.row_base, self.plan, self.D, self.R, self.d_concat, self.d_logit,
+                                                             -lr, self.table, self.lin_w, self.lin_bias, self.sum_x, self.x_sorted,
+                                                             self.lin_old_t, self.tab_amax, self.wg_ws[0], self.B, sc, dstW, dstb, wg_h2=True,
+                                                             parts=parts, refresh=tgt)
+            self._k("emb_pool_bwd_dups", "hbm", 0, lambda: dups(1))
+            if tgt is None:
+                refresh_planes_behind()
         else:
+            tgt = None
             self._k("emb_pool_bwd_dups", "hbm", 0, lambda: k4(1))
-        self._k("emb_hot_rows_apply", "hbm", 0, lambda: k4(2))
+        self._k("emb_hot_rows_apply", "hbm", 0, (lambda: dups(2)) if tgt is not None else (lambda: k4(2)))
         if not early:
             self._prefetch_issue(mark)
         self._k4_fused_done = True
diff --git a/deep_recommenders_amd/ops.py b/deep_recommenders_amd/ops.py
--- a/deep_recommenders_amd/ops.py
+++ b/deep_recommenders_amd/ops.py
@@ -525,7 +525,7 @@
     return plan
 
 
-def hash_sort_slots(keys, col_buckets, row_base, num_rows, ids_out, ids_t_out=None, plan=None):
+def hash_sort_slots(keys, col_buckets, row_base, num_rows, ids_out, ids_t_out=None, plan=None, parts=3):
     keys = _c(keys, torch.int64)
     B, F = keys.shape
     assert ids_out.shape == (B, F) and ids_out.dtype == torch.int64 and ids_out.is_contiguous()
@@ -533,6 +533,12 @@
         assert ids_t_out.shape == (F, B) and ids_t_out.dtype == torch.int32 and ids_t_out.is_contiguous()
     if plan is None or plan.n < B * F:
         plan = SortPlan(B * F, keys.device)
+    if parts != 3:
+        check(lib().dr_hash_sort_slots_parts(ptr(keys), B, F, ptr(col_buckets), ptr(ids_out), ptr(ids_t_out), ptr(row_base), int(num_rows),
+                                             ptr(plan.rows), ptr(plan.slots), ptr(plan.flags), ptr(plan.dup_heads), ptr(plan.dup_count),
+                                             ptr(plan.workspace), plan.workspace.numel(), int(parts), stream_ptr()),
+              "dr_hash_sort_slots_parts")
+        return plan
     check(lib().dr_hash_sort_slots(ptr(keys), B, F, ptr(col_buckets), ptr(ids_out), ptr(ids_t_out), ptr(row_base), int(num_rows),
                                    ptr(plan.rows), ptr(plan.slots), ptr(plan.flags), ptr(plan.dup_heads), ptr(plan.dup_count),
                                    ptr(plan.workspace), plan.workspace.numel(), stream_ptr()), "dr_hash_sort_slots")
@@ -574,12 +580,22 @@
 
 
 def emb_pool_bwd_dups_apply(ids, row_base, plan, D, num_rows, grad, d_fm_logit, scale, dst_table, dst_lin, dst_bias, sum_x, x_sorted,
-                            lin_old_t, table_amax, wg_workspace, wg_R, wg_scale, dstW, dstb=None, wg_h2=True, parts=1):
+                            lin_old_t, table_amax, wg_workspace, wg_R, wg_scale, dstW, dstb=None, wg_h2=True, parts=1, refresh=None):
     ids = _c(ids, torch.int64)
     B, F = ids.shape
     wg_F, wg_N = dstW.shape
     assert grad.stride(1) == 1 and dstW.stride(1) == 1
     assert lin_old_t is None or (lin_old_t.shape == (F, B) and lin_old_t.is_contiguous() and lin_old_t.dtype == torch.float32)
+    if refresh is not None:
+        w, wt, amax, words = refresh
+        assert (w.rows, w.cols) == (wg_F, wg_N) and (wt.rows, wt.cols) == (wg_N, wg_F) and words.numel() >= 1024
+        check(lib().dr_emb_pool_bwd_dups_apply_refresh(
+            ptr(ids), ptr(row_base), ptr(plan.rows), ptr(plan.slots), ptr(plan.flags), ptr(plan.dup_heads), ptr(plan.dup_count), B, F, D,
+            int(num_rows), ptr(grad), grad.stride(0), ptr(sum_x), ptr(d_fm_logit), float(scale), ptr(dst_table), ptr(dst_lin), ptr(dst_bias),
+            ptr(x_sorted), ptr(lin_old_t), int(parts) | 8, ptr(table_amax), ptr(wg_workspace), wg_workspace.numel() * 4, int(wg_R), wg_F,
+            wg_N, 1 if wg_h2 else 0, float(wg_scale), ptr(dstW), dstW.stride(0), ptr(dstb), ptr(w.buf), w.plane_stride, w.ld, ptr(wt.buf),
+            wt.plane_stride, wt.ld, ptr(amax), ptr(words), stream_ptr()), "dr_emb_pool_bwd_dups_apply_refresh")
+        return
     check(lib().dr_emb_pool_bwd_dups_apply(ptr(ids), ptr(row_base), ptr(plan.rows), ptr(plan.slots), ptr(plan.flags), ptr(plan.dup_heads),
                                            ptr(plan.dup_count), B, F, D, int(num_rows), ptr(grad), grad.stride(0), ptr(sum_x),
                                            ptr(d_fm_logit), float(scale), ptr(dst_table), ptr(dst_lin), ptr(dst_bias), ptr(x_sorted),
@@ -1342,16 +1358,27 @@
         self.w = H2Planes(K, N, W.device, self.amax)
         self._w_alt = H2Planes(K, N, W.device, h2_record(W.device)) if double_buffer else None
         self._parts = None
+        self._ride_words = None
         self.refresh()
+
+    def _swap(self):
+        if self._w_alt is not None:
+            self.w, self._w_alt = self._w_alt, self.w
+            self.amax = self.w.amax
+            self.wt.amax = self.amax
+
+    def hand_off(self):
+        if self._ride_words is None:
+            self._ride_words = torch.zeros(1024, dtype=torch.int32, device=self.W.device)
+        self._swap()
+        self._ver = self.W._version
+        return self.w, self.wt, self.amax, self._ride_words
 
     def refresh(self):
         if self._parts is None:
             self._parts = torch.zeros(256, dtype=torch.int32, device=self.W.device)
         K, N = self.W.shape
-        if self._w_alt is not None:
-            self.w, self._w_alt = self._w_alt, self.w
-            self.amax = self.w.amax
-            self.wt.amax = self.amax
+        self._swap()
         check(lib().dr_h2_refresh_weight(ptr(self.W), self.W.stride(0), K, N, ptr(self.w.buf), self.w.plane_stride, self.w.ld,
                                          ptr(self.wt.buf), self.wt.plane_stride, self.wt.ld, ptr(self.amax), ptr(self._parts),
                                          stream_ptr()), "dr_h2_refresh_weight")
diff --git a/include/dr_hotpath.h b/include/dr_hotpath.h
--- a/include/dr_hotpath.h
+++ b/include/dr_hotpath.h
@@ -70,6 +70,10 @@
                        int32_t* ids_t_out, const int64_t* row_base, int64_t num_rows, int64_t* sorted_rows,
                        int32_t* sorted_slots, uint8_t* unique_flags, int32_t* dup_heads, int32_t* dup_count, void* workspace,
                        int64_t workspace_bytes, dr_stream_t stream);
+int dr_hash_sort_slots_parts(const int64_t* keys, int64_t B, int32_t F, const uint64_t* col_buckets, int64_t* ids_out,
+                             int32_t* ids_t_out, const int64_t* row_base, int64_t num_rows, int64_t* sorted_rows,
+                             int32_t* sorted_slots, uint8_t* unique_flags, int32_t* dup_heads, int32_t* dup_count, void* workspace,
+                             int64_t workspace_bytes, int32_t parts, dr_stream_t stream);
 int dr_emb_pool_bwd_sorted(const int64_t* ids, const int64_t* row_base, const int64_t* sorted_rows,
                            const int32_t* sorted_slots, const uint8_t* unique_flags,
                            const int32_t* dup_heads, const int32_t* dup_count, int64_t B, int32_t F,
@@ -322,6 +326,15 @@
                                const float* lin_old_t, int32_t parts, uint32_t* table_amax, void* wg_workspace,
                                int64_t wg_workspace_bytes, int64_t wg_R, int32_t wg_F, int32_t wg_N, int32_t wg_h2, float wg_scale,
                                float* dstW, int64_t ld_w, float* dstb, dr_stream_t stream);
+int dr_emb_pool_bwd_dups_apply_refresh(const int64_t* ids, const int64_t* row_base, const int64_t* sorted_rows,
+                                       const int32_t* sorted_slots, const uint8_t* unique_flags, const int32_t* dup_heads,
+                                       const int32_t* dup_count, int64_t B, int32_t F, int32_t D, int64_t num_rows, const float* grad,
+                                       int64_t ld_grad, const float* sum_x, const float* d_fm_logit, float scale, float* dst_table,
+                                       float* dst_lin, float* dst_bias, float* x_sorted, const float* lin_old_t, int32_t parts,
+                                       uint32_t* table_amax, void* wg_workspace, int64_t wg_workspace_bytes, int64_t wg_R, int32_t wg_F,
+                                       int32_t wg_N, int32_t wg_h2, float wg_scale, float* dstW, int64_t ld_w, float* dstb,
+                                       void* w_planes, int64_t w_plane_stride, int64_t w_ld, void* wt_planes, int64_t wt_plane_stride,
+                                       int64_t wt_ld, uint32_t* w_amax, uint32_t* amax_parts, dr_stream_t stream);
 
 
 int dr_cin_fwd(const float* x0, const float* x, int64_t B, int32_t H0, int32_t Hk, int32_t D, const float* W,
```

Result: faster. 75.22 million examples/sec (median of 6 runs) (+3.7%).
